# yilundu/cross_attention_renderer

Hardware: AMD Instinct MI355X
Metric: rendered_rays_per_sec (higher is better)
Workload: dtype f32 (split-f16 x3 MFMA); 1 GPU; 256x256 query frame, 64 samples/view, 2 context views (config 2), a new query pose every step (cameras on the host), 1 forward call(s) x 1 scene(s) x 65536 rays per rank; builder_kept=False, H=256, samples_per_view=64, parallelism=one GPU

## Files before the change

### cross_attention_renderer_amd/csrc/car_raychain.hip

```cpp
#include "car_common.h"
#include "car_geom.h"

namespace {

typedef float f32x16 __attribute__((ext_vector_type(16)));
typedef _Float16 half8 __attribute__((ext_vector_type(8)));
typedef __fp16 fp16x2 __attribute__((ext_vector_type(2)));
typedef __attribute__((address_space(3))) void lds_void;

constexpr int kTileFloats = 1024;
constexpr int kMaxNT = 9;
constexpr int kBufFloats = kMaxNT * kTileFloats;
constexpr int kMaxChunks = 96;
constexpr int kMaxLayers = 16;

struct Chunk { unsigned off; int nt; };
struct ChainArgs {
    const float* arena;
    const float* bias;
    const float* scale;
    int layer[kMaxLayers];
    Chunk chunk[kMaxChunks];
    int n_chunks;
    const float* x0; int ld0;
    const float* x1; int ld1;
    const float* z1_in;
    float* out0;
    float* out1;
    const CarRay* rays;
    long M;
    int V, R;
    float zscale;
};

constexpr int kRing = 3;
struct Stream {
    const ChainArgs& a;
    float* lds;
    int g;
    __device__ __forceinline__ float* buffer(int gi) const { return lds + (gi % kRing) * kBufFloats; }
    __device__ __forceinline__ void issue(int gi, int tid, int wave) const {
        if (gi >= a.n_chunks) return;
        const Chunk c = a.chunk[gi];
        const float* src = a.arena + c.off;
        float* dst = buffer(gi);
        for (int t = 0; t < c.nt; ++t) {
            const unsigned lds_dst = __builtin_amdgcn_readfirstlane((unsigned)(uintptr_t)(lds_void*)(dst + 4 * (t * 256 + wave * 64)));
            const float* gsrc = src + 4 * (t * 256 + tid);
            unsigned keep;
            asm volatile("s_mov_b32 %0, m0\n\ts_mov_b32 m0, %2\n\ts_nop 0\n\tglobal_load_lds_dwordx4 %1, off\n\ts_mov_b32 m0, %0"
                         : "=&s"(keep) : "v"(gsrc), "s"(lds_dst) : "memory");
        }
    }
    __device__ __forceinline__ void landed(int gi) const {
        const int n = __builtin_amdgcn_readfirstlane(gi + 1 < a.n_chunks ? a.chunk[gi + 1].nt : 0);
        switch (n) {
            case 1: asm volatile("s_waitcnt vmcnt(1)" ::: "memory"); break;
            case 4: asm volatile("s_waitcnt vmcnt(4)" ::: "memory"); break;
            case 9: asm volatile("s_waitcnt vmcnt(9)" ::: "memory"); break;
            default: asm volatile("s_waitcnt vmcnt(0)" ::: "memory"); break;
        }
        __syncthreads();
    }
    __device__ __forceinline__ void sync() const { landed(g + 1); }
};

#include "car_split.h"
template <int NT>
__device__ __forceinline__ void scale(f32x16 (&acc)[NT], float f) {
#pragma unroll
    for (int t = 0; t < NT; ++t) acc[t] *= f;
}

template <int NT>
__device__ __forceinline__ void mma_chunk(f32x16 (&acc)[NT], const float* wl, const float (&x8)[2][8], float p) {
    half8 bhi[2], blo[2];
#pragma unroll
    for (int kg = 0; kg < 2; ++kg) split8(x8[kg], p, bhi[kg], blo[kg]);
    auto read = [&](int i, half8& ah, half8& al) {
        const int t = i >> 1, kg = i & 1;
        ah = __builtin_bit_cast(half8, *reinterpret_cast<const float4*>(wl + t * kTileFloats + ((kg * 2 + 0) * 64) * 4));
        al = __builtin_bit_cast(half8, *reinterpret_cast<const float4*>(wl + t * kTileFloats + ((kg * 2 + 1) * 64) * 4));
    };
    half8 ah[2], al[2];
    read(0, ah[0], al[0]);
#pragma unroll
    for (int i = 0; i < 2 * NT; ++i) {
        const int t = i >> 1, kg = i & 1, cur = i & 1;
        if (i + 1 < 2 * NT) read(i + 1, ah[cur ^ 1], al[cur ^ 1]);
        __builtin_amdgcn_sched_barrier(0);
        acc[t] = __builtin_amdgcn_mfma_f32_32x32x16_f16(ah[cur], bhi[kg], acc[t], 0, 0, 0);
        acc[t] = __builtin_amdgcn_mfma_f32_32x32x16_f16(ah[cur], blo[kg], acc[t], 0, 0, 0);
        acc[t] = __builtin_amdgcn_mfma_f32_32x32x16_f16(al[cur], bhi[kg], acc[t], 0, 0, 0);
        __builtin_amdgcn_sched_barrier(0);
    }
}

template <int NT>
__device__ __forceinline__ void layer_global(f32x16 (&acc)[NT], const float* xrow, int K, int chunks, float dW, Stream& st, int tid, int lane,
                                             int wave) {
    const int h = lane >> 5;
    auto load = [&](int c, float (&x8)[2][8]) {
#pragma unroll
        for (int kg = 0; kg < 2; ++kg) {
            const int k0 = 32 * c + 16 * kg + 8 * h;
#pragma unroll
            for (int q = 0; q < 2; ++q) {
                const int kq = k0 + 4 * q;
                const float4 v = *reinterpret_cast<const float4*>(xrow + (kq + 4 <= K ? kq : 0));
                const float e[4] = {v.x, v.y, v.z, v.w};
#pragma unroll
                for (int i = 0; i < 4; ++i) x8[kg][4 * q + i] = kq + 4 <= K ? e[i] : (kq + i < K ? xrow[kq + i] : 0.0f);
            }
        }
    };
    float m = 0.0f;
    for (int c = 0; c < chunks; ++c) {
        float x8[2][8];
        load(c, x8);
#pragma unroll
        for (int kg = 0; kg < 2; ++kg)
#pragma unroll
            for (int e = 0; e < 8; ++e) m = fmaxf(m, fabsf(x8[kg][e]));
    }
    m = fmaxf(m, __shfl_xor(m, 32, 64));
    float p, pinv;
    pow2_scale(fmaxf(m, 1e-30f), p, pinv);
    scale<NT>(acc, p / dW);
    float cur[2][8], nxt[2][8];
    load(0, cur);
    for (int c = 0; c < chunks; ++c) {
        st.issue(st.g + 2, tid, wave);
        if (c + 1 < chunks) load(c + 1, nxt);
        mma_chunk<NT>(acc, st.buffer(st.g) + 4 * lane, cur, p);
#pragma unroll
        for (int kg = 0; kg < 2; ++kg)
#pragma unroll
            for (int e = 0; e < 8; ++e) cur[kg][e] = nxt[kg][e];
        st.sync();
        ++st.g;
    }
    scale<NT>(acc, dW * pinv);
}
template <int NSRC, int NT, bool RELU>
__device__ __forceinline__ void layer_chained(f32x16 (&acc)[NT], const f32x16 (&src)[NSRC], float dW, Stream& st, int tid, int lane, int wave) {
    float m = 0.0f;
#pragma unroll
    for (int T = 0; T < NSRC; ++T)
#pragma unroll
        for (int r = 0; r < 16; ++r) m = fmaxf(m, RELU ? src[T][r] : fabsf(src[T][r]));
    m = fmaxf(m, __shfl_xor(m, 32, 64));
    float p, pinv;
    pow2_scale(fmaxf(m, 1e-30f), p, pinv);
    scale<NT>(acc, p / dW);
#pragma unroll
    for (int T = 0; T < NSRC; ++T) {
        st.issue(st.g + 2, tid, wave);
        float x8[2][8];
#pragma unroll
        for (int kg = 0; kg < 2; ++kg)
#pragma unroll
            for (int e = 0; e < 8; ++e) x8[kg][e] = RELU ? fmaxf(src[T][8 * kg + e], 0.0f) : src[T][8 * kg + e];
        mma_chunk<NT>(acc, st.buffer(st.g) + 4 * lane, x8, p);
        st.sync();
        ++st.g;
    }
    scale<NT>(acc, dW * pinv);
}
template <int NT>
__device__ __forceinline__ void add_bias(f32x16 (&acc)[NT], const float* b, int h) {
#pragma unroll
    for (int t = 0; t < NT; ++t)
#pragma unroll
        for (int r = 0; r < 16; ++r) acc[t][r] += b[32 * t + (r & 3) + 8 * (r >> 2) + 4 * h];
}
template <int NT>
__device__ __forceinline__ void zero(f32x16 (&acc)[NT]) {
#pragma unroll
    for (int t = 0; t < NT; ++t)
#pragma unroll
        for (int r = 0; r < 16; ++r) acc[t][r] = 0.0f;
}
template <int NT>
__device__ __forceinline__ void store_rows(const f32x16 (&acc)[NT], float* row, int N, int h) {
#pragma unroll
    for (int t = 0; t < NT; ++t)
#pragma unroll
        for (int g = 0; g < 4; ++g) {
            const int n0 = 32 * t + 8 * g + 4 * h;
            if (n0 + 4 <= N) *reinterpret_cast<float4*>(row + n0) = make_float4(acc[t][4 * g], acc[t][4 * g + 1], acc[t][4 * g + 2], acc[t][4 * g + 3]);
        }
}

__global__ void __launch_bounds__(256, 1) ray_mid_kernel(const ChainArgs a) {
    extern __shared__ __attribute__((aligned(16))) float lds[];
    const int tid = threadIdx.x, lane = tid & 63, wave = tid >> 6, s = lane & 31, h = lane >> 5;
    const long row = (long)blockIdx.x * 128 + wave * 32 + s;
    const long lrow = row < a.M ? row : a.M - 1;
    auto dW = [&](int i) { return a.scale[kMaxLayers + a.layer[i]]; };
    Stream st{a, lds, 0};
    st.issue(0, tid, wave);
    st.issue(1, tid, wave);
    st.landed(0);
    f32x16 z1[9];
    zero<9>(z1);
    add_bias<9>(z1, a.bias, h);
    layer_global<9>(z1, a.x0 + lrow * a.ld0, 576, 18, dW(0), st, tid, lane, wave);
    if (row < a.M) store_rows<9>(z1, a.out0 + row * 288, 288, h);
    f32x16 hb[4];
    zero<4>(hb);
    add_bias<4>(hb, a.bias + 288, h);
    layer_chained<9, 4, false>(hb, z1, dW(1), st, tid, lane, wave);
    f32x16 uh[4];
    zero<4>(uh);
    layer_chained<4, 4, false>(uh, hb, dW(2), st, tid, lane, wave);
    if (row < a.M) store_rows<4>(uh, a.out1 + row * 128, 128, h);
}

__global__ void __launch_bounds__(256, 1) ray_tail_kernel(const ChainArgs a) {
    extern __shared__ __attribute__((aligned(16))) float lds[];
    const int tid = threadIdx.x, lane = tid & 63, wave = tid >> 6, s = lane & 31, h = lane >> 5;
    const long row = (long)blockIdx.x * 128 + wave * 32 + s;
    const long lrow = row < a.M ? row : a.M - 1;
    auto dW = [&](int i) { return a.scale[kMaxLayers + a.layer[i]]; };
    Stream st{a, lds, 0};
    st.issue(0, tid, wave);
    st.issue(1, tid, wave);
    st.landed(0);
    f32x16 z[9];
#pragma unroll
    for (int t = 0; t < 9; ++t)
#pragma unroll
        for (int g = 0; g < 4; ++g) {
            const float4 v = *reinterpret_cast<const float4*>(a.z1_in + lrow * 288 + 32 * t + 8 * g + 4 * h);
            z[t][4 * g] = a.zscale * v.x; z[t][4 * g + 1] = a.zscale * v.y; z[t][4 * g + 2] = a.zscale * v.z; z[t][4 * g + 3] = a.zscale * v.w;
        }
    add_bias<9>(z, a.bias, h);
    layer_global<9>(z, a.x0 + lrow * a.ld0, 576, 18, dW(0), st, tid, lane, wave);
    const float* bias = a.bias + 288;
    f32x16 x[4], net[4];
    zero<4>(x);
    add_bias<4>(x, bias, h);
    layer_global<4>(x, a.x1 + lrow * a.ld1, 18, 1, dW(1), st, tid, lane, wave);
#pragma unroll
    for (int i = 0; i < 3; ++i) {
        add_bias<4>(x, bias + (3 * i + 1) * 128, h);
        layer_chained<9, 4, false>(x, z, dW(2 + 3 * i), st, tid, lane, wave);
        zero<4>(net);
        add_bias<4>(net, bias + (3 * i + 2) * 128, h);
        layer_chained<4, 4, true>(net, x, dW(3 + 3 * i), st, tid, lane, wave);
        add_bias<4>(x, bias + (3 * i + 3) * 128, h);
        layer_chained<4, 4, true>(x, net, dW(4 + 3 * i), st, tid, lane, wave);
    }
    f32x16 o[1];
    zero<1>(o);
    add_bias<1>(o, bias + 10 * 128, h);
    layer_chained<4, 1, true>(o, x, dW(11), st, tid, lane, wave);
    if (row < a.M && h == 0) {
        const long sc = row / a.R, r = row % a.R;
        float ov = 0.0f;
        for (int v = 0; v < a.V; ++v) ov = fmaxf(ov, a.rays[(sc * a.V + v) * a.R + r].overlaps);
        const float valid = ov > 0.0f ? 1.0f : 0.0f;
        for (int k = 0; k < 3; ++k) a.out0[3 * row + k] = o[0][k] * valid + (1.0f - valid);
        a.out1[row] = valid;
    }
}

__global__ void chain_scale_kernel(const float* __restrict__ W, int ldw, const float* __restrict__ W2, int K, int N, float* __restrict__ scale, int slot) {
    __shared__ float red[16];
    float m = 0.0f;
    for (long idx = threadIdx.x; idx < (long)N * K; idx += blockDim.x) {
        const long at = (idx / K) * ldw + idx % K;
        m = fmaxf(m, fabsf(W[at] + (W2 ? W2[at] : 0.0f)));
    }
    for (int o = 32; o > 0; o >>= 1) m = fmaxf(m, __shfl_xor(m, o, 64));
    if ((threadIdx.x & 63) == 0) red[threadIdx.x >> 6] = m;
    __syncthreads();
    if (threadIdx.x == 0) {
        for (int w = 1; w < (int)(blockDim.x / 64); ++w) m = fmaxf(m, red[w]);
        float p, inv;
        pow2_scale(fmaxf(m, 1e-30f), p, inv);
        scale[slot] = p;
        scale[kMaxLayers + slot] = inv;
    }
}
__global__ void pack_chain_kernel(const float* __restrict__ W, int ldw, const float* __restrict__ W2, int K, int N, int tiles, int chained,
                                  long total, const float* __restrict__ scale, int slot, _Float16* __restrict__ packed) {
    const float p = scale[slot];
    for (long idx = (long)blockIdx.x * blockDim.x + threadIdx.x; idx < total; idx += (long)gridDim.x * blockDim.x) {
        const int e = (int)(idx & 7), lane = (int)((idx >> 3) & 63), hl = (int)((idx >> 9) & 1), kg = (int)((idx >> 10) & 1);
        const long ct = idx >> 11;
        const int tile = (int)(ct % tiles), chunk = (int)(ct / tiles);
        const int n = 32 * tile + (lane & 31);
        const int k = chained ? 32 * chunk + (e & 3) + 8 * (2 * kg + (e >> 2)) + 4 * (lane >> 5) : 32 * chunk + 16 * kg + 8 * (lane >> 5) + e;
        float v = 0.0f;
        if (n < N && k < K) v = (W[(long)n * ldw + k] + (W2 ? W2[(long)n * ldw + k] : 0.0f)) * p;
        const _Float16 hi = (_Float16)v;
        packed[idx] = hl == 0 ? hi : (_Float16)(v - (float)hi);
    }
}

}

extern "C" size_t car_chain_packed_floats(int K, int N) { return (size_t)((K + 31) / 32) * ((N + 31) / 32) * kTileFloats; }
extern "C" int car_chain_pack(const float* W, int ldw, const float* W2, int K, int N, int chained, float* packed, float* scale, int slot,
                              void* stream) {
    CAR_REQUIRE(W && packed && scale && K > 0 && N > 0 && ldw >= K && slot >= 0 && slot < kMaxLayers, "car_chain_pack: bad arguments");
    const int tiles = (N + 31) / 32;
    const long total = (long)car_chain_packed_floats(K, N) * 2;
    (void)hipGetLastError();
    hipLaunchKernelGGL(chain_scale_kernel, dim3(1), dim3(1024), 0, (hipStream_t)stream, W, ldw, W2, K, N, scale, slot);
    hipLaunchKernelGGL(pack_chain_kernel, dim3(256), dim3(256), 0, (hipStream_t)stream, W, ldw, W2, K, N, tiles, chained, total, scale, slot,
                       reinterpret_cast<_Float16*>(packed));
    CAR_CHECK_LAUNCH("car_chain_pack");
    return CAR_OK;
}

namespace {
int launch_chain(bool tail, const float* arena, const unsigned* offs, const int* nts, int n_chunks, const float* bias, const float* scale,
                 const int* layers, int n_layers, const float* x0, int ld0, const float* x1, int ld1, const float* z1_in, float* out0, float* out1,
                 const float* rays, long M, int V, int R, float zscale, void* stream) {
    CAR_REQUIRE(n_chunks > 0 && n_chunks <= kMaxChunks && n_layers == (tail ? 12 : 3), "car_ray_chain: %d weight chunks, %d layers", n_chunks, n_layers);
    ChainArgs a;
    a.arena = arena; a.bias = bias; a.scale = scale; a.n_chunks = n_chunks;
    for (int i = 0; i < kMaxLayers; ++i) a.layer[i] = i < n_layers ? layers[i] : 0;
    for (int i = 0; i < n_layers; ++i) CAR_REQUIRE(layers[i] >= 0 && layers[i] < kMaxLayers, "car_ray_chain: bad scale slot");
    for (int i = 0; i < n_chunks; ++i) { a.chunk[i].off = offs[i]; a.chunk[i].nt = nts[i]; }
    a.x0 = x0; a.ld0 = ld0; a.x1 = x1; a.ld1 = ld1; a.z1_in = z1_in; a.out0 = out0; a.out1 = out1; a.rays = (const CarRay*)rays;
    a.M = M; a.V = V; a.R = R; a.zscale = zscale;
    const size_t lds_bytes = (size_t)kRing * kBufFloats * sizeof(float);
    auto kern = tail ? ray_tail_kernel : ray_mid_kernel;
    hipError_t e = hipFuncSetAttribute((const void*)kern, hipFuncAttributeMaxDynamicSharedMemorySize, (int)lds_bytes);
    if (e != hipSuccess) { car_set_error("car_ray_chain: cannot reserve LDS: %s", hipGetErrorString(e)); return CAR_E_LAUNCH; }
    (void)hipGetLastError();
    hipLaunchKernelGGL(kern, dim3(car_div_up(M, 128)), dim3(256), lds_bytes, (hipStream_t)stream, a);
    CAR_CHECK_LAUNCH("car_ray_chain");
    return CAR_OK;
}
}

extern "C" int car_ray_mid(const float* arena, const unsigned* offs, const int* nts, int n_chunks, const float* bias, const float* scale,
                           const int* layers, int n_layers, const float* ebar, int ld_ebar, float* z1, float* uh, long M, void* stream) {
    CAR_REQUIRE(arena && offs && nts && bias && scale && layers && ebar && z1 && uh && M > 0 && ld_ebar >= 576 && ld_ebar % 4 == 0,
                "car_ray_mid: bad arguments");
    return launch_chain(false, arena, offs, nts, n_chunks, bias, scale, layers, n_layers, ebar, ld_ebar, nullptr, 0, nullptr, z1, uh, nullptr, M, 0, 1,
                        0.0f, stream);
}
extern "C" int car_ray_tail(const float* arena, const unsigned* offs, const int* nts, int n_chunks, const float* bias, const float* scale,
                            const int* layers, int n_layers, const float* ebar, int ld_ebar, const float* phi_x, int ld_phi, const float* z1,
                            const float* rays, int b, int V, int R, float* rgb, float* valid, void* stream) {
    CAR_REQUIRE(arena && offs && nts && bias && scale && layers && ebar && phi_x && z1 && rays && rgb && valid, "car_ray_tail: null pointer");
    CAR_REQUIRE(b > 0 && V > 0 && R > 0 && ld_ebar >= 576 && ld_ebar % 4 == 0 && ld_phi >= 20 && ld_phi % 4 == 0, "car_ray_tail: bad sizes");
    return launch_chain(true, arena, offs, nts, n_chunks, bias, scale, layers, n_layers, ebar, ld_ebar, phi_x, ld_phi, z1, rgb, valid, rays, (long)b * R, V,
                        R, (float)V, stream);
}
```

### cross_attention_renderer_amd/csrc/car_render.hip

```cpp
#include "car_common.h"
#include "car_geom.h"
#include <math.h>
#include <string.h>
#include <vector>

namespace {

#include "car_fused_layout.h"

constexpr int kPhiIn = 18, kPhiLd = 20, kBlocks = 3;

inline size_t up64(size_t x) { return (x + 63) & ~(size_t)63; }

struct Plan {
    size_t steps, blob, fbias, wpt, r2qw, r2qb, proj[CAR_MAX_LEVELS], proj16[CAR_MAX_LEVELS], latent_value, lin_in, enc_c, qreh_c, lz_c[kBlocks], fc0_c[kBlocks],
        fc1_c[kBlocks], lout_c, chain_scale, mid_bias, tail_bias, total;
};
inline bool level_on_f16_pipe(int c) { return c % 4 == 0 && c >= 32; }
Plan plan_layout(const car_dims& d) {
    Plan p;
    size_t o = 0;
    auto take = [&](size_t n) { const size_t at = o; o += up64(n); return at; };
    p.steps = take((size_t)d.P);
    p.blob = take(car_fused_blob_floats());
    p.fbias = take(car_fused_bias_floats());
    p.wpt = take((size_t)kC * 4);
    p.r2qw = take(car_round2q_packed_floats());
    p.r2qb = take(car_round2q_bias_floats());
    for (int l = 0; l < CAR_MAX_LEVELS; ++l) p.proj[l] = l < d.n_levels ? take(car_linear_packed_floats(d.level_c[l], kC)) : 0;
    for (int l = 0; l < CAR_MAX_LEVELS; ++l) p.proj16[l] = (l < d.n_levels && level_on_f16_pipe(d.level_c[l])) ? take(car_linear_x3_packed_floats(d.level_c[l], kC)) : 0;
    p.latent_value = take(car_chain_packed_floats(kC, kE));
    p.lin_in = take(car_chain_packed_floats(kPhiIn, kD));
    p.enc_c = take(car_chain_packed_floats(kE, kD));
    p.qreh_c = take(car_chain_packed_floats(kD, kD));
    for (int i = 0; i < kBlocks; ++i) {
        p.lz_c[i] = take(car_chain_packed_floats(kE, kD));
        p.fc0_c[i] = take(car_chain_packed_floats(kD, kD));
        p.fc1_c[i] = take(car_chain_packed_floats(kD, kD));
    }
    p.lout_c = take(car_chain_packed_floats(kD, 3));
    p.chain_scale = take(32);
    p.mid_bias = take(kE + kD);
    p.tail_bias = take(kE + kD + 3 * kBlocks * kD + 32);
    p.total = o;
    return p;
}

int check_dims(const car_dims* d, const char* who) {
    CAR_REQUIRE(d, "%s: null dims", who);
    CAR_REQUIRE(d->b > 0 && d->R > 0 && d->P > 1 && d->H > 1 && d->W > 1, "%s: bad sizes", who);
    CAR_REQUIRE(d->V == 2 && d->n_levels == 3, "%s: the one-call forward covers n_view = 2 and three pyramid levels (got %d, %d); "
                "other configurations run through the stage entries", who, d->V, d->n_levels);
    int csum = 0;
    for (int l = 0; l < d->n_levels; ++l) {
        CAR_REQUIRE(d->level_h[l] > 0 && d->level_w[l] > 0 && d->level_c[l] > 0, "%s: bad level %d", who, l);
        csum += d->level_c[l];
    }
    CAR_REQUIRE(csum == kC, "%s: the levels' channels must add up to %d (got %d)", who, kC, csum);
    CAR_REQUIRE(2 * d->P <= 128 * 3, "%s: too many samples per ray", who);
    CAR_REQUIRE(car_lattice_of(*d).ok, "%s: every pyramid level must be an integer factor coarser than the widest one, the same factor in both "
                "directions (the fused kernel gathers them from their common lattice); other pyramids run through the stage entries", who);
    return CAR_OK;
}

struct Span { size_t off, cnt; };
struct Work {
    Span rays, phi_x, e, g, logit, logit2, pt, pixel_val, coords, at_wt, at_wt2, amax, depth, ebar, z1, uh, valid, part;
    size_t total;
};
const struct { const char* name; Span Work::*buf; } kFindable[] = {
    {"rays", &Work::rays}, {"e", &Work::e}, {"g", &Work::g}, {"logit", &Work::logit}, {"logit2", &Work::logit2}, {"pt", &Work::pt},
    {"at_wt2", &Work::at_wt2}, {"ebar", &Work::ebar}, {"z1", &Work::z1}, {"uh", &Work::uh}, {"part", &Work::part}};
inline size_t step_groups(const car_dims& d) { const int ts = car_fused_tile_steps(); return (size_t)((d.P + ts - 1) / ts); }
Work work_layout(const car_dims& d) {
    Work w;
    size_t o = 0;
    auto take = [&](size_t n) { const Span s{o, n}; o += up64(n); return s; };
    const size_t n = (size_t)d.b * d.V, S = n * d.R * d.P, BR = (size_t)d.b * d.R;
    w.rays = take(n * d.R * CAR_RAY_FLOATS);
    w.phi_x = take(BR * kPhiLd);
    w.e = take(S * kC);
    w.g = take(S * CAR_G_DIM);
    w.logit = take(S);
    w.logit2 = take(S);
    w.pt = take(S * 3);
    w.pixel_val = take(S * 2);
    w.coords = take(n * d.R * 9);
    w.at_wt = take(S);
    w.at_wt2 = take(S);
    w.amax = take(n * d.R);
    w.depth = take(BR);
    w.ebar = take(BR * kC);
    w.z1 = take(BR * kE);
    w.uh = take(BR * kD);
    w.valid = take(BR);
    w.part = take(n * d.R * step_groups(d) * kC);
    w.total = o;
    return w;
}

struct StageRec { const char* name; hipEvent_t start, stop; };
struct Profile {
    bool on = false;
    std::vector<StageRec> recs;
    std::vector<hipEvent_t> pool;
    hipEvent_t event() {
        if (!pool.empty()) { hipEvent_t e = pool.back(); pool.pop_back(); return e; }
        hipEvent_t e = nullptr;
        if (hipEventCreate(&e) != hipSuccess) e = nullptr;
        return e;
    }
    void clear() {
        for (StageRec& r : recs) { pool.push_back(r.start); pool.push_back(r.stop); }
        recs.clear();
    }
};
thread_local Profile g_prof;
struct Stage {
    hipStream_t st;
    bool live;
    Stage(const char* name, hipStream_t s) : st(s), live(g_prof.on) {
        if (!live) return;
        StageRec r{name, g_prof.event(), g_prof.event()};
        if (!r.start || !r.stop) { live = false; return; }
        (void)hipEventRecord(r.start, st);
        g_prof.recs.push_back(r);
    }
    ~Stage() { if (live) (void)hipEventRecord(g_prof.recs.back().stop, st); }
};

}

extern "C" void car_profile_enable(int on) { g_prof.clear(); g_prof.on = on != 0; }
extern "C" void car_profile_reset(void) { g_prof.clear(); }
extern "C" int car_profile_count(void) { return (int)g_prof.recs.size(); }
extern "C" int car_profile_read(int i, const char** name, float* ms) {
    CAR_REQUIRE(i >= 0 && i < (int)g_prof.recs.size() && name && ms, "car_profile_read: no stage %d", i);
    const StageRec& r = g_prof.recs[i];
    if (hipEventSynchronize(r.stop) != hipSuccess || hipEventElapsedTime(ms, r.start, r.stop) != hipSuccess) {
        car_set_error("car_profile_read: %s", hipGetErrorString(hipGetLastError()));
        return CAR_E_LAUNCH;
    }
    *name = r.name;
    return CAR_OK;
}

extern "C" void car_linspace(float a, float b, int n, float* out) {
    if (n == 1) { out[0] = a; return; }
    const float step = (b - a) / (float)(n - 1);
    const int half = n / 2;
    for (int i = 0; i < n; ++i) out[i] = i < half ? a + step * (float)i : b - step * (float)(n - 1 - i);
}

extern "C" size_t car_plan_bytes(const car_dims* dims) {
    if (check_dims(dims, "car_plan_bytes") != CAR_OK) return 0;
    return plan_layout(*dims).total * sizeof(float);
}
extern "C" size_t car_workspace_bytes(const car_dims* dims) {
    if (check_dims(dims, "car_workspace_bytes") != CAR_OK) return 0;
    return work_layout(*dims).total * sizeof(float);
}

namespace {
size_t lattice_floats(const car_dims& d) { const car_lattice L = car_lattice_of(d); return (size_t)d.b * d.V * 2 * L.h * L.w * kC; }
size_t level_floats(const car_dims& d, int l) { return (size_t)d.b * d.V * d.level_h[l] * d.level_w[l] * kC; }
size_t level_offset(const car_dims& d, int level) {
    size_t n = up64(lattice_floats(d)) + 64;
    for (int l = 0; l < level && l < d.n_levels; ++l) n += up64(level_floats(d, l));
    return n;
}
}
extern "C" size_t car_gmeta_offset(const car_dims* dims) {
    if (check_dims(dims, "car_gmeta_offset") != CAR_OK) return 0;
    return up64(lattice_floats(*dims));
}
extern "C" size_t car_gmaps_floats(const car_dims* dims) {
    if (check_dims(dims, "car_gmaps_floats") != CAR_OK) return 0;
    return level_offset(*dims, CAR_MAX_LEVELS + 1);
}
extern "C" int car_lattice_shape(const car_dims* dims, int* lat_h, int* lat_w, int* lat_pad) {
    CAR_TRY(check_dims(dims, "car_lattice_shape"));
    CAR_REQUIRE(lat_h && lat_w && lat_pad, "car_lattice_shape: null pointer");
    const car_lattice L = car_lattice_of(*dims);
    *lat_h = L.h; *lat_w = L.w; *lat_pad = L.pad;
    return CAR_OK;
}
extern "C" int car_workspace_find(const car_dims* dims, const char* name, size_t* offset_floats, size_t* n_floats) {
    CAR_TRY(check_dims(dims, "car_workspace_find"));
    CAR_REQUIRE(name && offset_floats && n_floats, "car_workspace_find: null pointer");
    const Work w = work_layout(*dims);
    for (const auto& t : kFindable)
        if (strcmp(t.name, name) == 0) { *offset_floats = (w.*t.buf).off; *n_floats = (w.*t.buf).cnt; return CAR_OK; }
    car_set_error("car_workspace_find: unknown tensor '%s'", name);
    return CAR_E_ARG;
}

extern "C" int car_plan_build(const car_dims* dims, const car_weights* w, void* plan, void* stream) {
    CAR_TRY(check_dims(dims, "car_plan_build"));
    CAR_REQUIRE(w && plan, "car_plan_build: null pointer");
    const float* const* all = reinterpret_cast<const float* const*>(w);
    for (size_t k = 0; k < sizeof(car_weights) / sizeof(const float*); ++k)
        CAR_REQUIRE(all[k], "car_plan_build: weight pointer %zu of car_weights is null", k);
    CAR_REQUIRE(car_fused_blob_floats() == (size_t)kBlobTiles * kTile && car_fused_bias_floats() == (size_t)(kBiasFloats + kBiasScratch),
                "car_plan_build: the fused kernel was built with another weight layout");
    const Plan p = plan_layout(*dims);
    float* base = static_cast<float*>(plan);
    hipStream_t st = (hipStream_t)stream;
    {
        float steps[1024];
        CAR_REQUIRE(dims->P <= 1024, "car_plan_build: P too large");
        car_linspace(0.0f, 1.0f, dims->P, steps);
        if (hipMemcpyAsync(base + p.steps, steps, sizeof(float) * dims->P, hipMemcpyHostToDevice, st) != hipSuccess ||
            hipStreamSynchronize(st) != hipSuccess) {
            car_set_error("car_plan_build: upload failed: %s", hipGetErrorString(hipGetLastError()));
            return CAR_E_LAUNCH;
        }
    }
    CAR_TRY(car_fused_pack(w, base + p.blob, base + p.fbias, base + p.wpt, stream));
    CAR_TRY(car_round2q_pack(w->query_repeat_embed_w, w->query_repeat_embed_b, w->query_repeat_embed_2_w, w->query_repeat_embed_2_b,
                             w->query_embed_w, w->query_embed_b, w->query_embed_2_w, w->query_embed_2_b, base + p.r2qw, base + p.r2qb, stream));
    int coff = 0;
    for (int l = 0; l < dims->n_levels; ++l) {
        CAR_TRY(car_linear_pack(w->query_encode_latent_w + coff, kC + 3, nullptr, dims->level_c[l], kC, base + p.proj[l], stream));
        if (level_on_f16_pipe(dims->level_c[l]))
            CAR_TRY(car_linear_x3_pack(w->query_encode_latent_w + coff, kC + 3, dims->level_c[l], kC, base + p.proj16[l], stream));
        coff += dims->level_c[l];
    }
    float* cs = base + p.chain_scale;
    CAR_TRY(car_chain_pack(w->latent_value_w, kC, nullptr, kC, kE, 0, base + p.latent_value, cs, 0, stream));
    CAR_TRY(car_chain_pack(w->encode_latent_w, kE, nullptr, kE, kD, 1, base + p.enc_c, cs, 1, stream));
    CAR_TRY(car_chain_pack(w->query_repeat_embed_w, kD + 16, nullptr, kD, kD, 1, base + p.qreh_c, cs, 2, stream));
    CAR_TRY(car_chain_pack(w->phi_lin_in_w, kPhiIn, nullptr, kPhiIn, kD, 0, base + p.lin_in, cs, 3, stream));
    for (int i = 0; i < kBlocks; ++i) {
        CAR_TRY(car_chain_pack(w->phi_lin_z_w[i], 2 * kE, w->phi_lin_z_w[i] + kE, kE, kD, 1, base + p.lz_c[i], cs, 4 + 3 * i, stream));
        CAR_TRY(car_chain_pack(w->phi_fc_0_w[i], kD, nullptr, kD, kD, 1, base + p.fc0_c[i], cs, 5 + 3 * i, stream));
        CAR_TRY(car_chain_pack(w->phi_fc_1_w[i], kD, nullptr, kD, kD, 1, base + p.fc1_c[i], cs, 6 + 3 * i, stream));
    }
    CAR_TRY(car_chain_pack(w->phi_lin_out_w, kD, nullptr, kD, 3, 1, base + p.lout_c, cs, 13, stream));
    const int tail_floats = kE + kD + 3 * kBlocks * kD + 32;
    if (hipMemsetAsync(base + p.tail_bias, 0, sizeof(float) * tail_floats, st) != hipSuccess) { car_set_error("car_plan_build: memset failed"); return CAR_E_LAUNCH; }
    auto d2d = [&](float* dst, const float* src, int n) { return hipMemcpyAsync(dst, src, sizeof(float) * n, hipMemcpyDeviceToDevice, st) == hipSuccess; };
    bool ok = d2d(base + p.mid_bias, w->latent_value_b, kE) && d2d(base + p.mid_bias + kE, w->encode_latent_b, kD);
    float* tb = base + p.tail_bias;
    ok = ok && d2d(tb, w->latent_value_b, kE) && d2d(tb + kE, w->phi_lin_in_b, kD);
    tb += kE + kD;
    for (int i = 0; i < kBlocks; ++i)
        ok = ok && d2d(tb + (3 * i + 0) * kD, w->phi_lin_z_b[i], kD) && d2d(tb + (3 * i + 1) * kD, w->phi_fc_0_b[i], kD) &&
             d2d(tb + (3 * i + 2) * kD, w->phi_fc_1_b[i], kD);
    ok = ok && d2d(tb + 3 * kBlocks * kD, w->phi_lin_out_b, 3);
    if (!ok) { car_set_error("car_plan_build: bias copy failed"); return CAR_E_LAUNCH; }
    return CAR_OK;
}

struct Plan16 { size_t blob, fbias, wpt, total; };
Plan16 plan16_layout() {
    Plan16 p;
    size_t o = 0;
    auto take = [&](size_t n) { const size_t at = o; o += up64(n); return at; };
    p.blob = take(car_fused_blob16_floats());
    p.fbias = take(car_fused_bias_floats());
    p.wpt = take((size_t)kC * 4);
    p.total = o;
    return p;
}
extern "C" size_t car_plan_f16_bytes(const car_dims* dims) {
    if (check_dims(dims, "car_plan_f16_bytes") != CAR_OK) return 0;
    return plan16_layout().total * sizeof(float);
}
extern "C" int car_plan_f16_build(const car_dims* dims, const car_weights* w, void* plan16, void* stream) {
    CAR_TRY(check_dims(dims, "car_plan_f16_build"));
    CAR_REQUIRE(w && plan16, "car_plan_f16_build: null pointer");
    CAR_REQUIRE(car_fused_blob16_floats() == (size_t)kBlobTiles * kTileHi && car_fused_bias_floats() == (size_t)(kBiasFloats + kBiasScratch),
                "car_plan_f16_build: the fused kernel was built with another weight layout");
    const Plan16 p = plan16_layout();
    float* base = static_cast<float*>(plan16);
    return car_fused_pack_hi(w, base + p.blob, base + p.fbias, base + p.wpt, stream);
}

extern "C" int car_project_maps(const car_dims* dims, const void* plan, const float* const* maps, float* gmaps, void* stream) {
    CAR_TRY(check_dims(dims, "car_project_maps"));
    CAR_REQUIRE(plan && maps && gmaps, "car_project_maps: null pointer");
    const Plan p = plan_layout(*dims);
    const float* base = static_cast<const float*>(plan);
    hipStream_t st = (hipStream_t)stream;
    float* gmeta = gmaps + car_gmeta_offset(dims);
    if (hipMemsetAsync(gmeta, 0, sizeof(float) * CAR_MAX_LEVELS, st) != hipSuccess) { car_set_error("car_project_maps: memset failed"); return CAR_E_LAUNCH; }
    const car_lattice L = car_lattice_of(*dims);
    const float* lv[CAR_MAX_LEVELS];
    for (int l = 0; l < dims->n_levels; ++l) {
        CAR_REQUIRE(maps[l], "car_project_maps: level %d is null", l);
        const long M = (long)dims->b * dims->V * dims->level_h[l] * dims->level_w[l];
        float* gl = gmaps + level_offset(*dims, l);
        if (level_on_f16_pipe(dims->level_c[l]) && ((uintptr_t)maps[l] & 15) == 0)
            CAR_TRY(car_linear_x3(maps[l], dims->level_c[l], base + p.proj16[l], nullptr, dims->level_c[l], kC, gl, kC, M, 0, stream));
        else
            CAR_TRY(car_linear(maps[l], dims->level_c[l], base + p.proj[l], dims->level_c[l], kC, gl, kC, M, 0, stream));
        lv[l] = gl;
    }
    return car_launch_merge(lv, dims->level_h, dims->level_w, L.r, dims->n_levels, L.h, L.w, L.pad, dims->b * dims->V, gmaps,
                            reinterpret_cast<unsigned*>(gmeta), st, "car_project_maps (merge)");
}

static int render_phases(const char* entry, const car_dims* dims, const void* plan, const car_inputs* in, const car_outputs* out,
                         void* workspace, size_t workspace_bytes, int phases, void* stream, const void* plan16 = nullptr) {
    const int which = phases & ~CAR_PHASE_ROWS_FIRST_ROUND;
    CAR_REQUIRE(which == CAR_PHASE_SAMPLES || which == CAR_PHASE_RAYS || which == (CAR_PHASE_SAMPLES | CAR_PHASE_RAYS),
                "%s: phases = %d (CAR_PHASE_SAMPLES, CAR_PHASE_RAYS or both, optionally | CAR_PHASE_ROWS_FIRST_ROUND)", entry, phases);
    CAR_TRY(check_dims(dims, "car_render_forward"));
    CAR_REQUIRE(plan && in && out && workspace, "car_render_forward: null pointer");
    CAR_REQUIRE(in->poses && in->uv && in->lattice && in->gmeta && out->rgb, "car_render_forward: poses, uv, lattice, gmeta and rgb are required");
    const car_dims& d = *dims;
    const Plan p = plan_layout(d);
    const Work w = work_layout(d);
    CAR_REQUIRE(workspace_bytes >= w.total * sizeof(float), "car_render_forward: workspace of %zu bytes, %zu needed", workspace_bytes,
                w.total * sizeof(float));
    const float* pl = static_cast<const float*>(plan);
    float* ws = static_cast<float*>(workspace);
    hipStream_t st = (hipStream_t)stream;
    const int b = d.b, V = d.V, R = d.R, P = d.P;
    const bool rows_first = (phases & CAR_PHASE_ROWS_FIRST_ROUND) != 0;
    CAR_REQUIRE(!d.no_sample || in->steps, "car_render_forward: no_sample needs `steps` (the P depths along the query ray, models.py:221-222)");
    const float* steps = in->steps ? in->steps : pl + p.steps;
    const long BR = (long)b * R;
    float* coords = out->coords ? out->coords : ws + w.coords.off;
    float* pixel_val = out->pixel_val ? out->pixel_val : ws + w.pixel_val.off;
    float* at_wt = out->at_wt ? out->at_wt : ws + w.at_wt.off;
    float* depth = out->depth_ray ? out->depth_ray : ws + w.depth.off;
    float* valid = out->valid_mask ? out->valid_mask : ws + w.valid.off;
    int32_t* amax = out->at_wt_max ? out->at_wt_max : reinterpret_cast<int32_t*>(ws + w.amax.off);

    if (phases & CAR_PHASE_SAMPLES) {
    {
        Stage stage("ray_setup", st);
        if (hipMemsetAsync(ws + w.phi_x.off, 0, sizeof(float) * BR * kPhiLd, st) != hipSuccess) { car_set_error("car_render_forward: memset failed"); return CAR_E_LAUNCH; }
        CAR_TRY(car_ray_setup(in->poses, in->uv, b, V, R, d.H, d.W, P, d.no_sample != 0, steps, ws + w.rays.off, coords, ws + w.phi_x.off, kPhiLd, stream));
    }
    {
        Stage stage("fused_samples", st);
        const car_lattice L = car_lattice_of(d);
        if (plan16) {
            const Plan16 q = plan16_layout();
            const float* p16 = static_cast<const float*>(plan16);
            CAR_TRY(car_fused_samples_f16(in->poses, ws + w.rays.off, steps, in->lattice, L.h, L.w, L.pad, in->gmeta, p16 + q.wpt, p16 + q.blob,
                                          p16 + q.fbias, b, V, R, P, d.H, d.W, d.no_sample != 0, ws + w.e.off, ws + w.g.off, ws + w.logit.off, ws + w.pt.off, pixel_val,
                                          rows_first ? nullptr : ws + w.part.off, stream));
        } else if (rows_first)
            CAR_TRY(car_fused_samples(in->poses, ws + w.rays.off, steps, in->lattice, L.h, L.w, L.pad, in->gmeta, pl + p.wpt, pl + p.blob,
                                      pl + p.fbias, b, V, R, P, d.H, d.W, d.no_sample != 0, ws + w.e.off, ws + w.g.off, ws + w.logit.off, ws + w.pt.off, pixel_val, stream));
        else
            CAR_TRY(car_fused_samples_parts(in->poses, ws + w.rays.off, steps, in->lattice, L.h, L.w, L.pad, in->gmeta, pl + p.wpt, pl + p.blob,
                                            pl + p.fbias, b, V, R, P, d.H, d.W, d.no_sample != 0, ws + w.e.off, ws + w.g.off, ws + w.logit.off, ws + w.pt.off, pixel_val,
                                            ws + w.part.off, stream));
    }
    }
    if (!(phases & CAR_PHASE_RAYS)) return CAR_OK;
    {
        Stage stage("attend_1", st);
        if (rows_first)
            CAR_TRY(car_attend(ws + w.logit.off, nullptr, kD, ws + w.e.off, kC, b, V, R, P, nullptr, 0.0f, at_wt, ws + w.ebar.off, kC, 1, ws + w.pt.off, in->poses,
                               depth, amax, stream));
        else
            CAR_TRY(car_attend_parts(ws + w.logit.off, ws + w.part.off, car_fused_tile_steps(), kC, b, V, R, P, at_wt, ws + w.ebar.off, kC, 1, ws + w.pt.off, in->poses,
                                     depth, amax, stream));
    }
    unsigned offs[96];
    int nts[96];
    int nch = 0;
    auto chunks = [&](size_t at, int n, int nt) { for (int c = 0; c < n; ++c) { offs[nch] = (unsigned)(at + (size_t)c * nt * 1024); nts[nch++] = nt; } };
    CAR_REQUIRE(p.total < (1ull << 32), "car_render_forward: plan too large");
    if (d.repeat_attention) {
        {
            Stage stage("ray_layers_1", st);
            nch = 0;
            chunks(p.latent_value, 18, 9); chunks(p.enc_c, 9, 4); chunks(p.qreh_c, 4, 4);
            const int layers[3] = {0, 1, 2};
            CAR_TRY(car_ray_mid(pl, offs, nts, nch, pl + p.mid_bias, pl + p.chain_scale, layers, 3, ws + w.ebar.off, kC, ws + w.z1.off, ws + w.uh.off, BR, stream));
        }
        {
            Stage stage("round2_logits", st);
            CAR_TRY(car_round2_logits_from_g(ws + w.g.off, ws + w.uh.off, pl + p.r2qw, pl + p.r2qb, b, V, R, P, ws + w.logit2.off, stream));
        }
        {
            Stage stage("attend_2", st);
            CAR_TRY(car_attend(ws + w.logit2.off, nullptr, kD, ws + w.e.off, kC, b, V, R, P, nullptr, 0.0f, ws + w.at_wt2.off, ws + w.ebar.off, kC, 1, nullptr,
                               nullptr, nullptr, nullptr, stream));
        }
    } else if (hipMemsetAsync(ws + w.z1.off, 0, sizeof(float) * BR * kE, st) != hipSuccess) {
        car_set_error("car_render_forward: memset failed");
        return CAR_E_LAUNCH;
    }
    {
        Stage stage("ray_layers_2", st);
        nch = 0;
        chunks(p.latent_value, 18, 9); chunks(p.lin_in, 1, 4);
        for (int i = 0; i < kBlocks; ++i) { chunks(p.lz_c[i], 9, 4); chunks(p.fc0_c[i], 4, 4); chunks(p.fc1_c[i], 4, 4); }
        chunks(p.lout_c, 4, 1);
        const int layers[12] = {0, 3, 4, 5, 6, 7, 8, 9, 10, 11, 12, 13};
        CAR_TRY(car_ray_tail(pl, offs, nts, nch, pl + p.tail_bias, pl + p.chain_scale, layers, 12, ws + w.ebar.off, kC, ws + w.phi_x.off, kPhiLd, ws + w.z1.off,
                             ws + w.rays.off, b, V, R, out->rgb, valid, stream));
    }
    return CAR_OK;
}

extern "C" int car_render_forward(const car_dims* dims, const void* plan, const car_inputs* in, const car_outputs* out,
                                  void* workspace, size_t workspace_bytes, void* stream) {
    return render_phases("car_render_forward", dims, plan, in, out, workspace, workspace_bytes, CAR_PHASE_SAMPLES | CAR_PHASE_RAYS, stream);
}

extern "C" int car_render_forward_phase(const car_dims* dims, const void* plan, const car_inputs* in, const car_outputs* out,
                                        void* workspace, size_t workspace_bytes, int phases, void* stream) {
    return render_phases("car_render_forward_phase", dims, plan, in, out, workspace, workspace_bytes, phases, stream);
}

extern "C" int car_render_forward_f16(const car_dims* dims, const void* plan, const void* plan16, const car_inputs* in, const car_outputs* out,
                                      void* workspace, size_t workspace_bytes, int phases, void* stream) {
    CAR_REQUIRE(plan16, "car_render_forward_f16: null plan16");
    return render_phases("car_render_forward_f16", dims, plan, in, out, workspace, workspace_bytes, phases, stream, plan16);
}
```

### cross_attention_renderer_amd/csrc/car_round2.hip

```cpp
#include "car_common.h"

namespace {

typedef float f32x16 __attribute__((ext_vector_type(16)));
typedef float f32x4 __attribute__((ext_vector_type(4)));
typedef _Float16 half8 __attribute__((ext_vector_type(8)));
typedef __fp16 fp16x2 __attribute__((ext_vector_type(2)));
constexpr int kD = 128, kNT = 4, kTile = 1024, kChunks = 4;
constexpr int kWaves = 8, kStageLd = 36;
constexpr int kLdsW1 = kChunks * kNT * kTile;
constexpr int kLdsBias = kLdsW1 + kNT * 512;
constexpr int kLdsStage = kLdsBias + 2 * kD + 4;
constexpr size_t kLdsBytes = (size_t)(kLdsStage + kWaves * 32 * kStageLd) * sizeof(float);
constexpr int kLdsWq1 = kLdsBias;
constexpr int kLdsBiasG = kLdsWq1 + kNT * 512;
constexpr int kBiasFloatsG = 4 * kD + 8;
constexpr int kScratchG = kD * kD;
constexpr size_t kLdsBytesG = (size_t)(kLdsBiasG + kBiasFloatsG) * sizeof(float);

#include "car_split.h"

template <bool ZERO = false>
__device__ __forceinline__ void first_layer(const half8& ghi, const half8& glo, const float* lw1, const float* lb1, float up, int lane, int h,
                                            f32x16 (&ug)[kNT]) {
#pragma unroll
    for (int t = 0; t < kNT; ++t) {
#pragma unroll
        for (int r = 0; r < 16; ++r) ug[t][r] = ZERO ? 0.0f : lb1[32 * t + (r & 3) + 8 * (r >> 2) + 4 * h] * up;
        const float* w1 = lw1 + t * 512 + 4 * lane;
        const half8 ah = __builtin_bit_cast(half8, *reinterpret_cast<const float4*>(w1));
        const half8 al = __builtin_bit_cast(half8, *reinterpret_cast<const float4*>(w1 + 256));
        ug[t] = __builtin_amdgcn_mfma_f32_32x32x16_f16(ah, ghi, ug[t], 0, 0, 0);
        ug[t] = __builtin_amdgcn_mfma_f32_32x32x16_f16(ah, glo, ug[t], 0, 0, 0);
        ug[t] = __builtin_amdgcn_mfma_f32_32x32x16_f16(al, ghi, ug[t], 0, 0, 0);
    }
}
template <bool ZERO = false>
__device__ __forceinline__ void second_layer(const f32x16 (&x)[kNT], float xp, const float* lw2, const float* lb2, float up2, int lane, int h,
                                             f32x16 (&acc)[kNT]) {
#pragma unroll
    for (int t = 0; t < kNT; ++t)
#pragma unroll
        for (int r = 0; r < 16; ++r) acc[t][r] = ZERO ? 0.0f : lb2[32 * t + (r & 3) + 8 * (r >> 2) + 4 * h] * up2;
#pragma unroll
    for (int c = 0; c < kChunks; ++c) {
        half8 bhi[2], blo[2];
#pragma unroll
        for (int kg = 0; kg < 2; ++kg) {
            float x8[8];
#pragma unroll
            for (int e = 0; e < 8; ++e) x8[e] = x[c][8 * kg + e];
            split8(x8, xp, bhi[kg], blo[kg]);
        }
        const float* wl = lw2 + c * kNT * kTile + 4 * lane;
        auto read = [&](int i, half8& ah, half8& al) {
            const int t = i >> 1, kg = i & 1;
            ah = __builtin_bit_cast(half8, *reinterpret_cast<const float4*>(wl + t * kTile + ((kg * 2 + 0) * 64) * 4));
            al = __builtin_bit_cast(half8, *reinterpret_cast<const float4*>(wl + t * kTile + ((kg * 2 + 1) * 64) * 4));
        };
        half8 ah[2], al[2];
        read(0, ah[0], al[0]);
#pragma unroll
        for (int i = 0; i < 2 * kNT; ++i) {
            const int t = i >> 1, kg = i & 1, cur = i & 1;
            if (i + 1 < 2 * kNT) read(i + 1, ah[cur ^ 1], al[cur ^ 1]);
            __builtin_amdgcn_sched_barrier(0);
            acc[t] = __builtin_amdgcn_mfma_f32_32x32x16_f16(ah[cur], bhi[kg], acc[t], 0, 0, 0);
            acc[t] = __builtin_amdgcn_mfma_f32_32x32x16_f16(ah[cur], blo[kg], acc[t], 0, 0, 0);
            acc[t] = __builtin_amdgcn_mfma_f32_32x32x16_f16(al[cur], bhi[kg], acc[t], 0, 0, 0);
            __builtin_amdgcn_sched_barrier(0);
        }
    }
}

template <bool G>
__global__ void __launch_bounds__(512) round2_kernel(const float* __restrict__ g, const float* __restrict__ uh,
                                                     const float* __restrict__ qry, const float* __restrict__ wpacked,
                                                     const float* __restrict__ bias, int V, int R, int P, long S,
                                                     float* __restrict__ logit) {
    extern __shared__ __attribute__((aligned(16))) float lds[];
    const int tid = threadIdx.x, lane = tid & 63, wave = tid >> 6;
    const int s = lane & 31, h = lane >> 5;
    const int qd = lane & 7, r8 = lane >> 3;
    constexpr int kW = G ? kLdsBiasG : kLdsBias, kB = G ? kBiasFloatsG : 2 * kD + 4;
    for (int k = tid; k < kW / 4; k += 512)
        *reinterpret_cast<float4*>(lds + 4 * k) = *reinterpret_cast<const float4*>(wpacked + 4 * k);
    for (int k = tid; k < kB; k += 512) lds[kW + k] = bias[k];
    __syncthreads();
    const float* lb = lds + kW;
    const float down1 = lb[(G ? 4 : 2) * kD], down2 = lb[(G ? 4 : 2) * kD + 1];
    float* stage = lds + kLdsStage + wave * 32 * kStageLd;

    for (long row0 = ((long)blockIdx.x * kWaves + wave) * 32; row0 < S; row0 += (long)gridDim.x * kWaves * 32) {
        float4 qs[G ? 1 : kChunks][G ? 1 : 4];
        if constexpr (!G) {
#pragma unroll
            for (int it = 0; it < 4; ++it) {
                const long row = row0 + r8 + 8 * it < S ? row0 + r8 + 8 * it : S - 1;
#pragma unroll
                for (int c = 0; c < kChunks; ++c) {
                    const f32x4 v = __builtin_nontemporal_load(reinterpret_cast<const f32x4*>(qry + row * kD + 32 * c + 4 * qd));
                    qs[c][it] = make_float4(v[0], v[1], v[2], v[3]);
                }
            }
        }
        const long srow = row0 + s < S ? row0 + s : S - 1;
        const long nr = srow / P;
        const float* uhrow = uh + (((nr / R) / V) * R + nr % R) * kD;
        half8 ghi, glo;
        float gp, ginv;
        {
            const float4 g0 = *reinterpret_cast<const float4*>(g + srow * 16 + 8 * h);
            const float4 g1 = *reinterpret_cast<const float4*>(g + srow * 16 + 8 * h + 4);
            const float gx[8] = {g0.x, g0.y, g0.z, g0.w, g1.x, g1.y, g1.z, g1.w};
            float m = 0.0f;
#pragma unroll
            for (int k = 0; k < 8; ++k) m = fmaxf(m, fabsf(gx[k]));
            m = fmaxf(m, __shfl_xor(m, 32, 64));
            pow2_scale(fmaxf(m, 1e-30f), gp, ginv);
            split8(gx, gp, ghi, glo);
        }
        f32x16 ug[kNT];
        first_layer<G>(ghi, glo, lds + kLdsW1, lb, gp / down1, lane, h, ug);
        const float undo1 = down1 * ginv;
        float xm = 0.0f;
#pragma unroll
        for (int t = 0; t < kNT; ++t)
#pragma unroll
            for (int gq = 0; gq < 4; ++gq) {
                const float4 u = *reinterpret_cast<const float4*>(uhrow + 32 * t + 8 * gq + 4 * h);
                float uu[4] = {u.x, u.y, u.z, u.w};
                if constexpr (G) {
                    const float4 b = *reinterpret_cast<const float4*>(lb + 32 * t + 8 * gq + 4 * h);
                    uu[0] += b.x; uu[1] += b.y; uu[2] += b.z; uu[3] += b.w;
                }
#pragma unroll
                for (int r = 0; r < 4; ++r) {
                    const float x = fmaxf(fmaf(ug[t][4 * gq + r], undo1, uu[r]), 0.0f);
                    ug[t][4 * gq + r] = x;
                    xm = fmaxf(xm, x);
                }
            }
        float dot = 0.0f;
        if constexpr (G) {
            const float downq = lb[4 * kD + 2];
            f32x16 xq[kNT];
            first_layer<true>(ghi, glo, lds + kLdsWq1, lb + 2 * kD, gp / downq, lane, h, xq);
            const float undoq = downq * ginv;
            const float* lu = lb + 3 * kD;
            const float* lq = lb + 2 * kD;
            float xqm = 0.0f, dot_u = 0.0f;
#pragma unroll
            for (int t = 0; t < kNT; ++t)
#pragma unroll
                for (int gq = 0; gq < 4; ++gq) {
                    const float4 u = *reinterpret_cast<const float4*>(lu + 32 * t + 8 * gq + 4 * h);
                    const float4 b = *reinterpret_cast<const float4*>(lq + 32 * t + 8 * gq + 4 * h);
                    const float uu[4] = {u.x, u.y, u.z, u.w}, bb[4] = {b.x, b.y, b.z, b.w};
#pragma unroll
                    for (int r = 0; r < 4; ++r) {
                        const float x = fmaxf(fmaf(xq[t][4 * gq + r], undoq, bb[r]), 0.0f);
                        xq[t][4 * gq + r] = x;
                        xqm = fmaxf(xqm, x);
                        dot_u = fmaf(uu[r], x, dot_u);
                    }
                }
            xqm = fmaxf(xqm, __shfl_xor(xqm, 32, 64));
            float xp, xinv;
            pow2_scale(fmaxf(xqm, 1e-30f), xp, xinv);
            f32x16 acc[kNT];
            second_layer<true>(xq, xp, lds, lb + kD, xp / down2, lane, h, acc);
            const float* lv = lb + kD;
            float dot_v = 0.0f;
#pragma unroll
            for (int t = 0; t < kNT; ++t)
#pragma unroll
                for (int gq = 0; gq < 4; ++gq) {
                    const float4 v4 = *reinterpret_cast<const float4*>(lv + 32 * t + 8 * gq + 4 * h);
                    const float vv[4] = {v4.x, v4.y, v4.z, v4.w};
#pragma unroll
                    for (int r = 0; r < 4; ++r) {
                        dot = fmaf(ug[t][4 * gq + r], acc[t][4 * gq + r], dot);
                        dot_v = fmaf(ug[t][4 * gq + r], vv[r], dot_v);
                    }
                }
            dot = fmaf(dot, down2 * xinv, dot_u + dot_v);
            dot += __shfl_xor(dot, 32, 64);
            dot += lb[4 * kD + 3];
        } else {
            xm = fmaxf(xm, __shfl_xor(xm, 32, 64));
            float xp, xinv;
            pow2_scale(fmaxf(xm, 1e-30f), xp, xinv);
            f32x16 acc[kNT];
            second_layer(ug, xp, lds, lb + kD, xp / down2, lane, h, acc);
#pragma unroll
            for (int t = 0; t < kNT; ++t) {
#pragma unroll
                for (int it = 0; it < 4; ++it) *reinterpret_cast<float4*>(stage + (r8 + 8 * it) * kStageLd + 4 * qd) = qs[t][it];
#pragma unroll
                for (int gq = 0; gq < 4; ++gq) {
                    const float4 qv = *reinterpret_cast<const float4*>(stage + s * kStageLd + 8 * gq + 4 * h);
                    dot = fmaf(acc[t][4 * gq + 0], qv.x, dot); dot = fmaf(acc[t][4 * gq + 1], qv.y, dot);
                    dot = fmaf(acc[t][4 * gq + 2], qv.z, dot); dot = fmaf(acc[t][4 * gq + 3], qv.w, dot);
                }
            }
            dot += __shfl_xor(dot, 32, 64);
            dot *= down2 * xinv;
        }
        if (h == 0 && row0 + s < S) logit[row0 + s] = dot / 16.0f;
    }
}

}

extern "C" size_t car_round2_packed_floats(void) { return (size_t)kLdsBias; }
extern "C" size_t car_round2_bias_floats(void) { return (size_t)(2 * kD + 4); }

extern "C" size_t car_round2q_packed_floats(void) { return (size_t)kLdsBiasG; }
extern "C" size_t car_round2q_bias_floats(void) { return (size_t)(kBiasFloatsG + kScratchG); }

static int launch_round2(bool qg, const float* g, const float* uh, const float* qry, const float* wpacked, const float* bias,
                         int b, int V, int R, int P, float* logit, void* stream, const char* who) {
    CAR_REQUIRE(g && uh && (qg || qry) && wpacked && bias && logit, "%s: null pointer", who);
    CAR_REQUIRE(b > 0 && V > 0 && R > 0 && P > 0, "%s: bad sizes", who);
    const long S = (long)b * V * R * P;
    void (*kern)(const float*, const float*, const float*, const float*, const float*, int, int, int, long, float*) =
        qg ? round2_kernel<true> : round2_kernel<false>;
    const size_t lds_bytes = qg ? kLdsBytesG : kLdsBytes;
    hipError_t e = hipFuncSetAttribute((const void*)kern, hipFuncAttributeMaxDynamicSharedMemorySize, (int)lds_bytes);
    if (e != hipSuccess) { car_set_error("%s: cannot reserve LDS: %s", who, hipGetErrorString(e)); return CAR_E_LAUNCH; }
    const long groups = (S + 255) / 256;
    const unsigned blocks = (unsigned)(groups < 1024 ? groups : 1024);
    (void)hipGetLastError();
    hipLaunchKernelGGL(kern, dim3(blocks), dim3(512), lds_bytes, (hipStream_t)stream, g, uh, qry, wpacked, bias, V, R, P, S, logit);
    hipError_t e_ = hipGetLastError();
    if (e_ != hipSuccess) { car_set_error("%s: launch failed: %s", who, hipGetErrorString(e_)); return CAR_E_LAUNCH; }
    return CAR_OK;
}

extern "C" int car_round2_logits(const float* g, const float* uh, const float* qry, const float* wpacked, const float* bias,
                                 int b, int V, int R, int P, float* logit, void* stream) {
    return launch_round2(false, g, uh, qry, wpacked, bias, b, V, R, P, logit, stream, "car_round2_logits");
}

extern "C" int car_round2_logits_from_g(const float* g, const float* uh, const float* wpacked, const float* bias, int b, int V, int R, int P,
                                        float* logit, void* stream) {
    return launch_round2(true, g, uh, nullptr, wpacked, bias, b, V, R, P, logit, stream, "car_round2_logits_from_g");
}
```

Before: 2.154 million rays/s.

## Switch ray chain to 16x16 MFMA tiles with 8 waves and restructure round2 query path

Result: no change. 2.161 million rays/s (median of 4 runs) (+0.3%).

```diff
diff --git a/cross_attention_renderer_amd/csrc/car_raychain.hip b/cross_attention_renderer_amd/csrc/car_raychain.hip
--- a/cross_attention_renderer_amd/csrc/car_raychain.hip
+++ b/cross_attention_renderer_amd/csrc/car_raychain.hip
@@ -3,13 +3,14 @@
 
 namespace {
 
-typedef float f32x16 __attribute__((ext_vector_type(16)));
+typedef float f32x4 __attribute__((ext_vector_type(4)));
 typedef _Float16 half8 __attribute__((ext_vector_type(8)));
 typedef __fp16 fp16x2 __attribute__((ext_vector_type(2)));
 typedef __attribute__((address_space(3))) void lds_void;
 
-constexpr int kTileFloats = 1024;
-constexpr int kMaxNT = 9;
+constexpr int kTileFloats = 512;
+constexpr int kMaxNT = 18;
+constexpr int kWaves = 8, kWaveRays = 16, kGroupRays = kWaves * kWaveRays;
 constexpr int kBufFloats = kMaxNT * kTileFloats;
 constexpr int kMaxChunks = 96;
 constexpr int kMaxLayers = 16;
@@ -38,26 +39,30 @@
     const ChainArgs& a;
     float* lds;
     int g;
+    int wave;
     __device__ __forceinline__ float* buffer(int gi) const { return lds + (gi % kRing) * kBufFloats; }
-    __device__ __forceinline__ void issue(int gi, int tid, int wave) const {
+    __device__ __forceinline__ int wave_loads(int gi, int wave) const { return gi < a.n_chunks ? (2 * a.chunk[gi].nt - wave + kWaves - 1) / kWaves : 0; }
+    __device__ __forceinline__ void issue(int gi, int lane, int wave) const {
         if (gi >= a.n_chunks) return;
         const Chunk c = a.chunk[gi];
         const float* src = a.arena + c.off;
         float* dst = buffer(gi);
-        for (int t = 0; t < c.nt; ++t) {
-            const unsigned lds_dst = __builtin_amdgcn_readfirstlane((unsigned)(uintptr_t)(lds_void*)(dst + 4 * (t * 256 + wave * 64)));
-            const float* gsrc = src + 4 * (t * 256 + tid);
+        for (int j = wave; j < 2 * c.nt; j += kWaves) {
+            const unsigned lds_dst = __builtin_amdgcn_readfirstlane((unsigned)(uintptr_t)(lds_void*)(dst + 4 * (j * 64)));
+            const float* gsrc = src + 4 * (j * 64 + lane);
             unsigned keep;
             asm volatile("s_mov_b32 %0, m0\n\ts_mov_b32 m0, %2\n\ts_nop 0\n\tglobal_load_lds_dwordx4 %1, off\n\ts_mov_b32 m0, %0"
                          : "=&s"(keep) : "v"(gsrc), "s"(lds_dst) : "memory");
         }
     }
     __device__ __forceinline__ void landed(int gi) const {
-        const int n = __builtin_amdgcn_readfirstlane(gi + 1 < a.n_chunks ? a.chunk[gi + 1].nt : 0);
+        const int n = __builtin_amdgcn_readfirstlane(wave_loads(gi + 1, wave));
         switch (n) {
             case 1: asm volatile("s_waitcnt vmcnt(1)" ::: "memory"); break;
+            case 2: asm volatile("s_waitcnt vmcnt(2)" ::: "memory"); break;
+            case 3: asm volatile("s_waitcnt vmcnt(3)" ::: "memory"); break;
             case 4: asm volatile("s_waitcnt vmcnt(4)" ::: "memory"); break;
-            case 9: asm volatile("s_waitcnt vmcnt(9)" ::: "memory"); break;
+            case 5: asm volatile("s_waitcnt vmcnt(5)" ::: "memory"); break;
             default: asm volatile("s_waitcnt vmcnt(0)" ::: "memory"); break;
         }
         __syncthreads();
@@ -67,100 +72,97 @@
 
 #include "car_split.h"
 template <int NT>
-__device__ __forceinline__ void scale(f32x16 (&acc)[NT], float f) {
+__device__ __forceinline__ void scale(f32x4 (&acc)[NT], float f) {
 #pragma unroll
     for (int t = 0; t < NT; ++t) acc[t] *= f;
 }
 
 template <int NT>
-__device__ __forceinline__ void mma_chunk(f32x16 (&acc)[NT], const float* wl, const float (&x8)[2][8], float p) {
-    half8 bhi[2], blo[2];
-#pragma unroll
-    for (int kg = 0; kg < 2; ++kg) split8(x8[kg], p, bhi[kg], blo[kg]);
-    auto read = [&](int i, half8& ah, half8& al) {
-        const int t = i >> 1, kg = i & 1;
-        ah = __builtin_bit_cast(half8, *reinterpret_cast<const float4*>(wl + t * kTileFloats + ((kg * 2 + 0) * 64) * 4));
-        al = __builtin_bit_cast(half8, *reinterpret_cast<const float4*>(wl + t * kTileFloats + ((kg * 2 + 1) * 64) * 4));
+__device__ __forceinline__ void mma_chunk(f32x4 (&acc)[NT], const float* wl, const float (&x8)[8], float p) {
+    half8 bhi, blo;
+    split8(x8, p, bhi, blo);
+    auto read = [&](int t, half8& ah, half8& al) {
+        ah = __builtin_bit_cast(half8, *reinterpret_cast<const float4*>(wl + t * kTileFloats));
+        al = __builtin_bit_cast(half8, *reinterpret_cast<const float4*>(wl + t * kTileFloats + 256));
     };
-    half8 ah[2], al[2];
+    half8 ah[3], al[3];
     read(0, ah[0], al[0]);
-#pragma unroll
-    for (int i = 0; i < 2 * NT; ++i) {
-        const int t = i >> 1, kg = i & 1, cur = i & 1;
-        if (i + 1 < 2 * NT) read(i + 1, ah[cur ^ 1], al[cur ^ 1]);
+    if (NT > 1) read(1, ah[1], al[1]);
+#pragma unroll
+    for (int t = 0; t < NT; ++t) {
+        const int cur = t % 3;
+        if (t + 2 < NT) read(t + 2, ah[(t + 2) % 3], al[(t + 2) % 3]);
         __builtin_amdgcn_sched_barrier(0);
-        acc[t] = __builtin_amdgcn_mfma_f32_32x32x16_f16(ah[cur], bhi[kg], acc[t], 0, 0, 0);
-        acc[t] = __builtin_amdgcn_mfma_f32_32x32x16_f16(ah[cur], blo[kg], acc[t], 0, 0, 0);
-        acc[t] = __builtin_amdgcn_mfma_f32_32x32x16_f16(al[cur], bhi[kg], acc[t], 0, 0, 0);
+        acc[t] = __builtin_amdgcn_mfma_f32_16x16x32_f16(ah[cur], bhi, acc[t], 0, 0, 0);
+        acc[t] = __builtin_amdgcn_mfma_f32_16x16x32_f16(ah[cur], blo, acc[t], 0, 0, 0);
+        acc[t] = __builtin_amdgcn_mfma_f32_16x16x32_f16(al[cur], bhi, acc[t], 0, 0, 0);
         __builtin_amdgcn_sched_barrier(0);
     }
 }
-
-template <int NT>
-__device__ __forceinline__ void layer_global(f32x16 (&acc)[NT], const float* xrow, int K, int chunks, float dW, Stream& st, int tid, int lane,
-                                             int wave) {
-    const int h = lane >> 5;
-    auto load = [&](int c, float (&x8)[2][8]) {
-#pragma unroll
-        for (int kg = 0; kg < 2; ++kg) {
-            const int k0 = 32 * c + 16 * kg + 8 * h;
-#pragma unroll
-            for (int q = 0; q < 2; ++q) {
-                const int kq = k0 + 4 * q;
-                const float4 v = *reinterpret_cast<const float4*>(xrow + (kq + 4 <= K ? kq : 0));
-                const float e[4] = {v.x, v.y, v.z, v.w};
-#pragma unroll
-                for (int i = 0; i < 4; ++i) x8[kg][4 * q + i] = kq + 4 <= K ? e[i] : (kq + i < K ? xrow[kq + i] : 0.0f);
-            }
+__device__ __forceinline__ float ray_max(float m) {
+    m = fmaxf(m, __shfl_xor(m, 16, 64));
+    return fmaxf(m, __shfl_xor(m, 32, 64));
+}
+
+template <int NT>
+__device__ __forceinline__ void layer_global(f32x4 (&acc)[NT], const float* xrow, int K, int chunks, float dW, Stream& st, int lane) {
+    const int q = lane >> 4;
+    auto load = [&](int c, float (&x8)[8]) {
+        const int k0 = 32 * c + 8 * q;
+#pragma unroll
+        for (int j = 0; j < 2; ++j) {
+            const int kq = k0 + 4 * j;
+            const float4 v = *reinterpret_cast<const float4*>(xrow + (kq + 4 <= K ? kq : 0));
+            const float e[4] = {v.x, v.y, v.z, v.w};
+#pragma unroll
+            for (int i = 0; i < 4; ++i) x8[4 * j + i] = kq + 4 <= K ? e[i] : (kq + i < K ? xrow[kq + i] : 0.0f);
         }
     };
     float m = 0.0f;
     for (int c = 0; c < chunks; ++c) {
-        float x8[2][8];
+        float x8[8];
         load(c, x8);
 #pragma unroll
-        for (int kg = 0; kg < 2; ++kg)
-#pragma unroll
-            for (int e = 0; e < 8; ++e) m = fmaxf(m, fabsf(x8[kg][e]));
-    }
-    m = fmaxf(m, __shfl_xor(m, 32, 64));
+        for (int e = 0; e < 8; ++e) m = fmaxf(m, fabsf(x8[e]));
+    }
+    m = ray_max(m);
     float p, pinv;
     pow2_scale(fmaxf(m, 1e-30f), p, pinv);
     scale<NT>(acc, p / dW);
-    float cur[2][8], nxt[2][8];
+    float cur[8], nxt[8];
     load(0, cur);
     for (int c = 0; c < chunks; ++c) {
-        st.issue(st.g + 2, tid, wave);
+        st.issue(st.g + 2, lane, st.wave);
         if (c + 1 < chunks) load(c + 1, nxt);
         mma_chunk<NT>(acc, st.buffer(st.g) + 4 * lane, cur, p);
 #pragma unroll
-        for (int kg = 0; kg < 2; ++kg)
-#pragma unroll
-            for (int e = 0; e < 8; ++e) cur[kg][e] = nxt[kg][e];
+        for (int e = 0; e < 8; ++e) cur[e] = nxt[e];
         st.sync();
         ++st.g;
     }
     scale<NT>(acc, dW * pinv);
 }
 template <int NSRC, int NT, bool RELU>
-__device__ __forceinline__ void layer_chained(f32x16 (&acc)[NT], const f32x16 (&src)[NSRC], float dW, Stream& st, int tid, int lane, int wave) {
+__device__ __forceinline__ void layer_chained(f32x4 (&acc)[NT], const f32x4 (&src)[NSRC], float dW, Stream& st, int lane) {
+    static_assert(NSRC % 2 == 0, "a K step takes two source tiles");
     float m = 0.0f;
 #pragma unroll
     for (int T = 0; T < NSRC; ++T)
 #pragma unroll
-        for (int r = 0; r < 16; ++r) m = fmaxf(m, RELU ? src[T][r] : fabsf(src[T][r]));
-    m = fmaxf(m, __shfl_xor(m, 32, 64));
+        for (int r = 0; r < 4; ++r) m = fmaxf(m, RELU ? src[T][r] : fabsf(src[T][r]));
+    m = ray_max(m);
     float p, pinv;
     pow2_scale(fmaxf(m, 1e-30f), p, pinv);
     scale<NT>(acc, p / dW);
 #pragma unroll
-    for (int T = 0; T < NSRC; ++T) {
-        st.issue(st.g + 2, tid, wave);
-        float x8[2][8];
-#pragma unroll
-        for (int kg = 0; kg < 2; ++kg)
-#pragma unroll
-            for (int e = 0; e < 8; ++e) x8[kg][e] = RELU ? fmaxf(src[T][8 * kg + e], 0.0f) : src[T][8 * kg + e];
+    for (int c = 0; c < NSRC / 2; ++c) {
+        st.issue(st.g + 2, lane, st.wave);
+        float x8[8];
+#pragma unroll
+        for (int e = 0; e < 8; ++e) {
+            const float v = src[2 * c + (e >> 2)][e & 3];
+            x8[e] = RELU ? fmaxf(v, 0.0f) : v;
+        }
         mma_chunk<NT>(acc, st.buffer(st.g) + 4 * lane, x8, p);
         st.sync();
         ++st.g;
@@ -168,95 +170,89 @@
     scale<NT>(acc, dW * pinv);
 }
 template <int NT>
-__device__ __forceinline__ void add_bias(f32x16 (&acc)[NT], const float* b, int h) {
+__device__ __forceinline__ void add_bias(f32x4 (&acc)[NT], const float* b, int q) {
+#pragma unroll
+    for (int t = 0; t < NT; ++t) {
+        const float4 v = *reinterpret_cast<const float4*>(b + 16 * t + 4 * q);
+        acc[t][0] += v.x; acc[t][1] += v.y; acc[t][2] += v.z; acc[t][3] += v.w;
+    }
+}
+template <int NT>
+__device__ __forceinline__ void zero(f32x4 (&acc)[NT]) {
 #pragma unroll
     for (int t = 0; t < NT; ++t)
 #pragma unroll
-        for (int r = 0; r < 16; ++r) acc[t][r] += b[32 * t + (r & 3) + 8 * (r >> 2) + 4 * h];
-}
-template <int NT>
-__device__ __forceinline__ void zero(f32x16 (&acc)[NT]) {
-#pragma unroll
-    for (int t = 0; t < NT; ++t)
-#pragma unroll
-        for (int r = 0; r < 16; ++r) acc[t][r] = 0.0f;
-}
-template <int NT>
-__device__ __forceinline__ void store_rows(const f32x16 (&acc)[NT], float* row, int N, int h) {
-#pragma unroll
-    for (int t = 0; t < NT; ++t)
-#pragma unroll
-        for (int g = 0; g < 4; ++g) {
-            const int n0 = 32 * t + 8 * g + 4 * h;
-            if (n0 + 4 <= N) *reinterpret_cast<float4*>(row + n0) = make_float4(acc[t][4 * g], acc[t][4 * g + 1], acc[t][4 * g + 2], acc[t][4 * g + 3]);
-        }
-}
-
-__global__ void __launch_bounds__(256, 1) ray_mid_kernel(const ChainArgs a) {
+        for (int r = 0; r < 4; ++r) acc[t][r] = 0.0f;
+}
+template <int NT>
+__device__ __forceinline__ void store_rows(const f32x4 (&acc)[NT], float* row, int q) {
+#pragma unroll
+    for (int t = 0; t < NT; ++t) *reinterpret_cast<float4*>(row + 16 * t + 4 * q) = make_float4(acc[t][0], acc[t][1], acc[t][2], acc[t][3]);
+}
+
+__global__ void __launch_bounds__(64 * kWaves) ray_mid_kernel(const ChainArgs a) {
     extern __shared__ __attribute__((aligned(16))) float lds[];
-    const int tid = threadIdx.x, lane = tid & 63, wave = tid >> 6, s = lane & 31, h = lane >> 5;
-    const long row = (long)blockIdx.x * 128 + wave * 32 + s;
+    const int tid = threadIdx.x, lane = tid & 63, wave = __builtin_amdgcn_readfirstlane(tid >> 6), s = lane & 15, q = lane >> 4;
+    const long row = (long)blockIdx.x * kGroupRays + wave * kWaveRays + s;
     const long lrow = row < a.M ? row : a.M - 1;
     auto dW = [&](int i) { return a.scale[kMaxLayers + a.layer[i]]; };
-    Stream st{a, lds, 0};
-    st.issue(0, tid, wave);
-    st.issue(1, tid, wave);
+    Stream st{a, lds, 0, wave};
+    st.issue(0, lane, wave);
+    st.issue(1, lane, wave);
     st.landed(0);
-    f32x16 z1[9];
-    zero<9>(z1);
-    add_bias<9>(z1, a.bias, h);
-    layer_global<9>(z1, a.x0 + lrow * a.ld0, 576, 18, dW(0), st, tid, lane, wave);
-    if (row < a.M) store_rows<9>(z1, a.out0 + row * 288, 288, h);
-    f32x16 hb[4];
-    zero<4>(hb);
-    add_bias<4>(hb, a.bias + 288, h);
-    layer_chained<9, 4, false>(hb, z1, dW(1), st, tid, lane, wave);
-    f32x16 uh[4];
-    zero<4>(uh);
-    layer_chained<4, 4, false>(uh, hb, dW(2), st, tid, lane, wave);
-    if (row < a.M) store_rows<4>(uh, a.out1 + row * 128, 128, h);
-}
-
-__global__ void __launch_bounds__(256, 1) ray_tail_kernel(const ChainArgs a) {
+    f32x4 z1[18];
+    zero<18>(z1);
+    add_bias<18>(z1, a.bias, q);
+    layer_global<18>(z1, a.x0 + lrow * a.ld0, 576, 18, dW(0), st, lane);
+    if (row < a.M) store_rows<18>(z1, a.out0 + row * 288, q);
+    f32x4 hb[8];
+    zero<8>(hb);
+    add_bias<8>(hb, a.bias + 288, q);
+    layer_chained<18, 8, false>(hb, z1, dW(1), st, lane);
+    f32x4 uh[8];
+    zero<8>(uh);
+    layer_chained<8, 8, false>(uh, hb, dW(2), st, lane);
+    if (row < a.M) store_rows<8>(uh, a.out1 + row * 128, q);
+}
+
+__global__ void __launch_bounds__(64 * kWaves) ray_tail_kernel(const ChainArgs a) {
     extern __shared__ __attribute__((aligned(16))) float lds[];
-    const int tid = threadIdx.x, lane = tid & 63, wave = tid >> 6, s = lane & 31, h = lane >> 5;
-    const long row = (long)blockIdx.x * 128 + wave * 32 + s;
+    const int tid = threadIdx.x, lane = tid & 63, wave = __builtin_amdgcn_readfirstlane(tid >> 6), s = lane & 15, q = lane >> 4;
+    const long row = (long)blockIdx.x * kGroupRays + wave * kWaveRays + s;
     const long lrow = row < a.M ? row : a.M - 1;
     auto dW = [&](int i) { return a.scale[kMaxLayers + a.layer[i]]; };
-    Stream st{a, lds, 0};
-    st.issue(0, tid, wave);
-    st.issue(1, tid, wave);
+    Stream st{a, lds, 0, wave};
+    st.issue(0, lane, wave);
+    st.issue(1, lane, wave);
     st.landed(0);
-    f32x16 z[9];
-#pragma unroll
-    for (int t = 0; t < 9; ++t)
-#pragma unroll
-        for (int g = 0; g < 4; ++g) {
-            const float4 v = *reinterpret_cast<const float4*>(a.z1_in + lrow * 288 + 32 * t + 8 * g + 4 * h);
-            z[t][4 * g] = a.zscale * v.x; z[t][4 * g + 1] = a.zscale * v.y; z[t][4 * g + 2] = a.zscale * v.z; z[t][4 * g + 3] = a.zscale * v.w;
-        }
-    add_bias<9>(z, a.bias, h);
-    layer_global<9>(z, a.x0 + lrow * a.ld0, 576, 18, dW(0), st, tid, lane, wave);
+    f32x4 z[18];
+#pragma unroll
+    for (int t = 0; t < 18; ++t) {
+        const float4 v = *reinterpret_cast<const float4*>(a.z1_in + lrow * 288 + 16 * t + 4 * q);
+        z[t][0] = a.zscale * v.x; z[t][1] = a.zscale * v.y; z[t][2] = a.zscale * v.z; z[t][3] = a.zscale * v.w;
+    }
+    add_bias<18>(z, a.bias, q);
+    layer_global<18>(z, a.x0 + lrow * a.ld0, 576, 18, dW(0), st, lane);
     const float* bias = a.bias + 288;
-    f32x16 x[4], net[4];
-    zero<4>(x);
-    add_bias<4>(x, bias, h);
-    layer_global<4>(x, a.x1 + lrow * a.ld1, 18, 1, dW(1), st, tid, lane, wave);
-#pragma unroll
+    f32x4 x[8], net[8];
+    zero<8>(x);
+    add_bias<8>(x, bias, q);
+    layer_global<8>(x, a.x1 + lrow * a.ld1, 18, 1, dW(1), st, lane);
+#pragma unroll 1
     for (int i = 0; i < 3; ++i) {
-        add_bias<4>(x, bias + (3 * i + 1) * 128, h);
-        layer_chained<9, 4, false>(x, z, dW(2 + 3 * i), st, tid, lane, wave);
-        zero<4>(net);
-        add_bias<4>(net, bias + (3 * i + 2) * 128, h);
-        layer_chained<4, 4, true>(net, x, dW(3 + 3 * i), st, tid, lane, wave);
-        add_bias<4>(x, bias + (3 * i + 3) * 128, h);
-        layer_chained<4, 4, true>(x, net, dW(4 + 3 * i), st, tid, lane, wave);
-    }
-    f32x16 o[1];
+        add_bias<8>(x, bias + (3 * i + 1) * 128, q);
+        layer_chained<18, 8, false>(x, z, dW(2 + 3 * i), st, lane);
+        zero<8>(net);
+        add_bias<8>(net, bias + (3 * i + 2) * 128, q);
+        layer_chained<8, 8, true>(net, x, dW(3 + 3 * i), st, lane);
+        add_bias<8>(x, bias + (3 * i + 3) * 128, q);
+        layer_chained<8, 8, true>(x, net, dW(4 + 3 * i), st, lane);
+    }
+    f32x4 o[1];
     zero<1>(o);
-    add_bias<1>(o, bias + 10 * 128, h);
-    layer_chained<4, 1, true>(o, x, dW(11), st, tid, lane, wave);
-    if (row < a.M && h == 0) {
+    add_bias<1>(o, bias + 10 * 128, q);
+    layer_chained<8, 1, true>(o, x, dW(11), st, lane);
+    if (row < a.M && q == 0) {
         const long sc = row / a.R, r = row % a.R;
         float ov = 0.0f;
         for (int v = 0; v < a.V; ++v) ov = fmaxf(ov, a.rays[(sc * a.V + v) * a.R + r].overlaps);
@@ -288,11 +284,11 @@
                                   long total, const float* __restrict__ scale, int slot, _Float16* __restrict__ packed) {
     const float p = scale[slot];
     for (long idx = (long)blockIdx.x * blockDim.x + threadIdx.x; idx < total; idx += (long)gridDim.x * blockDim.x) {
-        const int e = (int)(idx & 7), lane = (int)((idx >> 3) & 63), hl = (int)((idx >> 9) & 1), kg = (int)((idx >> 10) & 1);
-        const long ct = idx >> 11;
+        const int e = (int)(idx & 7), lane = (int)((idx >> 3) & 63), hl = (int)((idx >> 9) & 1);
+        const long ct = idx >> 10;
         const int tile = (int)(ct % tiles), chunk = (int)(ct / tiles);
-        const int n = 32 * tile + (lane & 31);
-        const int k = chained ? 32 * chunk + (e & 3) + 8 * (2 * kg + (e >> 2)) + 4 * (lane >> 5) : 32 * chunk + 16 * kg + 8 * (lane >> 5) + e;
+        const int n = 16 * tile + (lane & 15);
+        const int k = chained ? 32 * chunk + 16 * (e >> 2) + 4 * (lane >> 4) + (e & 3) : 32 * chunk + 8 * (lane >> 4) + e;
         float v = 0.0f;
         if (n < N && k < K) v = (W[(long)n * ldw + k] + (W2 ? W2[(long)n * ldw + k] : 0.0f)) * p;
         const _Float16 hi = (_Float16)v;
@@ -302,11 +298,11 @@
 
 }
 
-extern "C" size_t car_chain_packed_floats(int K, int N) { return (size_t)((K + 31) / 32) * ((N + 31) / 32) * kTileFloats; }
+extern "C" size_t car_chain_packed_floats(int K, int N) { return (size_t)((K + 31) / 32) * ((N + 15) / 16) * kTileFloats; }
 extern "C" int car_chain_pack(const float* W, int ldw, const float* W2, int K, int N, int chained, float* packed, float* scale, int slot,
                               void* stream) {
     CAR_REQUIRE(W && packed && scale && K > 0 && N > 0 && ldw >= K && slot >= 0 && slot < kMaxLayers, "car_chain_pack: bad arguments");
-    const int tiles = (N + 31) / 32;
+    const int tiles = (N + 15) / 16;
     const long total = (long)car_chain_packed_floats(K, N) * 2;
     (void)hipGetLastError();
     hipLaunchKernelGGL(chain_scale_kernel, dim3(1), dim3(1024), 0, (hipStream_t)stream, W, ldw, W2, K, N, scale, slot);
@@ -325,7 +321,10 @@
     a.arena = arena; a.bias = bias; a.scale = scale; a.n_chunks = n_chunks;
     for (int i = 0; i < kMaxLayers; ++i) a.layer[i] = i < n_layers ? layers[i] : 0;
     for (int i = 0; i < n_layers; ++i) CAR_REQUIRE(layers[i] >= 0 && layers[i] < kMaxLayers, "car_ray_chain: bad scale slot");
-    for (int i = 0; i < n_chunks; ++i) { a.chunk[i].off = offs[i]; a.chunk[i].nt = nts[i]; }
+    for (int i = 0; i < n_chunks; ++i) {
+        CAR_REQUIRE(nts[i] > 0 && nts[i] <= kMaxNT, "car_ray_chain: chunk %d has %d tiles", i, nts[i]);
+        a.chunk[i].off = offs[i]; a.chunk[i].nt = nts[i];
+    }
     a.x0 = x0; a.ld0 = ld0; a.x1 = x1; a.ld1 = ld1; a.z1_in = z1_in; a.out0 = out0; a.out1 = out1; a.rays = (const CarRay*)rays;
     a.M = M; a.V = V; a.R = R; a.zscale = zscale;
     const size_t lds_bytes = (size_t)kRing * kBufFloats * sizeof(float);
@@ -333,7 +332,7 @@
     hipError_t e = hipFuncSetAttribute((const void*)kern, hipFuncAttributeMaxDynamicSharedMemorySize, (int)lds_bytes);
     if (e != hipSuccess) { car_set_error("car_ray_chain: cannot reserve LDS: %s", hipGetErrorString(e)); return CAR_E_LAUNCH; }
     (void)hipGetLastError();
-    hipLaunchKernelGGL(kern, dim3(car_div_up(M, 128)), dim3(256), lds_bytes, (hipStream_t)stream, a);
+    hipLaunchKernelGGL(kern, dim3(car_div_up(M, kGroupRays)), dim3(64 * kWaves), lds_bytes, (hipStream_t)stream, a);
     CAR_CHECK_LAUNCH("car_ray_chain");
     return CAR_OK;
 }
diff --git a/cross_attention_renderer_amd/csrc/car_render.hip b/cross_attention_renderer_amd/csrc/car_render.hip
--- a/cross_attention_renderer_amd/csrc/car_render.hip
+++ b/cross_attention_renderer_amd/csrc/car_render.hip
@@ -366,13 +366,13 @@
     unsigned offs[96];
     int nts[96];
     int nch = 0;
-    auto chunks = [&](size_t at, int n, int nt) { for (int c = 0; c < n; ++c) { offs[nch] = (unsigned)(at + (size_t)c * nt * 1024); nts[nch++] = nt; } };
+    auto chunks = [&](size_t at, int n, int nt) { for (int c = 0; c < n; ++c) { offs[nch] = (unsigned)(at + (size_t)c * nt * 512); nts[nch++] = nt; } };
     CAR_REQUIRE(p.total < (1ull << 32), "car_render_forward: plan too large");
     if (d.repeat_attention) {
         {
             Stage stage("ray_layers_1", st);
             nch = 0;
-            chunks(p.latent_value, 18, 9); chunks(p.enc_c, 9, 4); chunks(p.qreh_c, 4, 4);
+            chunks(p.latent_value, 18, 18); chunks(p.enc_c, 9, 8); chunks(p.qreh_c, 4, 8);
             const int layers[3] = {0, 1, 2};
             CAR_TRY(car_ray_mid(pl, offs, nts, nch, pl + p.mid_bias, pl + p.chain_scale, layers, 3, ws + w.ebar.off, kC, ws + w.z1.off, ws + w.uh.off, BR, stream));
         }
@@ -392,8 +392,8 @@
     {
         Stage stage("ray_layers_2", st);
         nch = 0;
-        chunks(p.latent_value, 18, 9); chunks(p.lin_in, 1, 4);
-        for (int i = 0; i < kBlocks; ++i) { chunks(p.lz_c[i], 9, 4); chunks(p.fc0_c[i], 4, 4); chunks(p.fc1_c[i], 4, 4); }
+        chunks(p.latent_value, 18, 18); chunks(p.lin_in, 1, 8);
+        for (int i = 0; i < kBlocks; ++i) { chunks(p.lz_c[i], 9, 8); chunks(p.fc0_c[i], 4, 8); chunks(p.fc1_c[i], 4, 8); }
         chunks(p.lout_c, 4, 1);
         const int layers[12] = {0, 3, 4, 5, 6, 7, 8, 9, 10, 11, 12, 13};
         CAR_TRY(car_ray_tail(pl, offs, nts, nch, pl + p.tail_bias, pl + p.chain_scale, layers, 12, ws + w.ebar.off, kC, ws + w.phi_x.off, kPhiLd, ws + w.z1.off,
diff --git a/cross_attention_renderer_amd/csrc/car_round2.hip b/cross_attention_renderer_amd/csrc/car_round2.hip
--- a/cross_attention_renderer_amd/csrc/car_round2.hip
+++ b/cross_attention_renderer_amd/csrc/car_round2.hip
@@ -70,6 +70,166 @@
             acc[t] = __builtin_amdgcn_mfma_f32_32x32x16_f16(al[cur], bhi[kg], acc[t], 0, 0, 0);
             __builtin_amdgcn_sched_barrier(0);
         }
+    }
+}
+
+template <class Shadow>
+__device__ __forceinline__ void second_layer_tile(const half8 (&bhi)[kChunks][2], const half8 (&blo)[kChunks][2], const float* lw2, int t, int lane, f32x16& acc,
+                                                  Shadow&& shadow) {
+    const float* wl = lw2 + t * kTile + 4 * lane;
+    auto read = [&](int i, half8& ah, half8& al) {
+        const int c = i >> 1, kg = i & 1;
+        ah = __builtin_bit_cast(half8, *reinterpret_cast<const float4*>(wl + c * kNT * kTile + ((kg * 2 + 0) * 64) * 4));
+        al = __builtin_bit_cast(half8, *reinterpret_cast<const float4*>(wl + c * kNT * kTile + ((kg * 2 + 1) * 64) * 4));
+    };
+    half8 ah[2], al[2];
+    read(0, ah[0], al[0]);
+    f32x16 a = {0.0f, 0.0f, 0.0f, 0.0f, 0.0f, 0.0f, 0.0f, 0.0f, 0.0f, 0.0f, 0.0f, 0.0f, 0.0f, 0.0f, 0.0f, 0.0f};
+#pragma unroll
+    for (int i = 0; i < 2 * kChunks; ++i) {
+        const int c = i >> 1, kg = i & 1, cur = i & 1;
+        if (i + 1 < 2 * kChunks) read(i + 1, ah[cur ^ 1], al[cur ^ 1]);
+        __builtin_amdgcn_sched_barrier(0);
+        a = __builtin_amdgcn_mfma_f32_32x32x16_f16(ah[cur], bhi[c][kg], a, 0, 0, 0);
+        __builtin_amdgcn_sched_barrier(0);
+        shadow(3 * i);
+        __builtin_amdgcn_sched_barrier(0);
+        a = __builtin_amdgcn_mfma_f32_32x32x16_f16(ah[cur], blo[c][kg], a, 0, 0, 0);
+        __builtin_amdgcn_sched_barrier(0);
+        shadow(3 * i + 1);
+        __builtin_amdgcn_sched_barrier(0);
+        a = __builtin_amdgcn_mfma_f32_32x32x16_f16(al[cur], bhi[c][kg], a, 0, 0, 0);
+        __builtin_amdgcn_sched_barrier(0);
+        shadow(3 * i + 2);
+        __builtin_amdgcn_sched_barrier(0);
+    }
+    acc = a;
+}
+
+typedef const __attribute__((address_space(3))) float lds_float;
+template <class Ptr>
+__device__ __forceinline__ void load4(Ptr p, float (&v)[4]) {
+    const f32x4 q = *(const f32x4*)p;
+    v[0] = q[0]; v[1] = q[1]; v[2] = q[2]; v[3] = q[3];
+}
+__device__ __forceinline__ void load4(lds_float* p, float (&v)[4]) {
+    const f32x4 q = *(const __attribute__((address_space(3))) f32x4*)p;
+    v[0] = q[0]; v[1] = q[1]; v[2] = q[2]; v[3] = q[3];
+}
+
+__device__ __forceinline__ void round2_g_tiles(const float* __restrict__ g, const float* __restrict__ uh, const float* lds, int V, int R, int P, long S,
+                                               float* __restrict__ logit, int lane, long first, long stride) {
+    const int s = lane & 31, h = lane >> 5;
+    const float* lb = lds + kLdsBiasG;
+    const float down1 = lb[4 * kD], down2 = lb[4 * kD + 1], downq = lb[4 * kD + 2];
+    unsigned lane_tables = (unsigned)(uintptr_t)(lds_float*)(lb + 4 * h);
+    asm volatile("" : "+v"(lane_tables));
+    lds_float* lbh = (lds_float*)(uintptr_t)lane_tables;
+    lds_float* lvh = lbh + kD;
+    lds_float* lqh = lbh + 2 * kD;
+    lds_float* luh = lbh + 3 * kD;
+    const bool narrow = S <= 0x7fffffffL;
+    auto sample = [&](long r0) { return r0 + s < S ? r0 + s : S - 1; };
+    auto uh_row = [&](long srow) {
+        if (narrow) {
+            const unsigned nr = (unsigned)srow / (unsigned)P;
+            return uh + ((size_t)((nr / (unsigned)R) / (unsigned)V) * (unsigned)R + nr % (unsigned)R) * kD;
+        }
+        const long nr = srow / P;
+        return uh + (((nr / R) / V) * R + nr % R) * kD;
+    };
+    if (first >= S) return;
+    long srow = sample(first);
+    float4 g0 = *reinterpret_cast<const float4*>(g + srow * 16 + 8 * h), g1 = *reinterpret_cast<const float4*>(g + srow * 16 + 8 * h + 4);
+    const float* uhrow = uh_row(srow);
+    float un[4][4];
+#pragma unroll
+    for (int gq = 0; gq < 4; ++gq) load4(uhrow + 8 * gq + 4 * h, un[gq]);
+    for (long row0 = first; row0 < S; row0 += stride) {
+        const long nsrow = sample(row0 + stride);
+        const float4 ng0 = *reinterpret_cast<const float4*>(g + nsrow * 16 + 8 * h), ng1 = *reinterpret_cast<const float4*>(g + nsrow * 16 + 8 * h + 4);
+        const float* nuhrow = uh_row(nsrow);
+        half8 ghi, glo;
+        float gp, ginv;
+        {
+            const float gx[8] = {g0.x, g0.y, g0.z, g0.w, g1.x, g1.y, g1.z, g1.w};
+            float m = 0.0f;
+#pragma unroll
+            for (int k = 0; k < 8; ++k) m = fmaxf(m, fabsf(gx[k]));
+            m = fmaxf(m, __shfl_xor(m, 32, 64));
+            pow2_scale(fmaxf(m, 1e-30f), gp, ginv);
+            split8(gx, gp, ghi, glo);
+        }
+        f32x16 xq[kNT];
+        first_layer<true>(ghi, glo, lds + kLdsWq1, lb, gp / downq, lane, h, xq);
+        const float undoq = downq * ginv;
+        float xqm = 0.0f, dot_u = 0.0f;
+#pragma unroll
+        for (int t = 0; t < kNT; ++t)
+#pragma unroll
+            for (int gq = 0; gq < 4; ++gq) {
+                float uu[4], bb[4];
+                load4(luh + 32 * t + 8 * gq, uu);
+                load4(lqh + 32 * t + 8 * gq, bb);
+#pragma unroll
+                for (int r = 0; r < 4; ++r) {
+                    const float x = fmaxf(fmaf(xq[t][4 * gq + r], undoq, bb[r]), 0.0f);
+                    xq[t][4 * gq + r] = x;
+                    xqm = fmaxf(xqm, x);
+                    dot_u = fmaf(uu[r], x, dot_u);
+                }
+            }
+        xqm = fmaxf(xqm, __shfl_xor(xqm, 32, 64));
+        float xp, xinv;
+        pow2_scale(fmaxf(xqm, 1e-30f), xp, xinv);
+        half8 bhi[kChunks][2], blo[kChunks][2];
+#pragma unroll
+        for (int c = 0; c < kChunks; ++c)
+#pragma unroll
+            for (int kg = 0; kg < 2; ++kg) {
+                float x8[8];
+#pragma unroll
+                for (int e = 0; e < 8; ++e) x8[e] = xq[c][8 * kg + e];
+                split8(x8, xp, bhi[c][kg], blo[c][kg]);
+            }
+        f32x16 ug[kNT];
+        first_layer<true>(ghi, glo, lds + kLdsW1, lb, gp / down1, lane, h, ug);
+        const float undo1 = down1 * ginv;
+        float dot = 0.0f, dot_v = 0.0f;
+        f32x16 prev;
+#pragma unroll
+        for (int t = 0; t < kNT; ++t) {
+            const float* unext = t + 1 < kNT ? uhrow + 32 * (t + 1) : nuhrow;
+            float b4[4][4], v4[4][4];
+            load4(lbh + 32 * t, b4[0]);
+            load4(lvh + 32 * t, v4[0]);
+            f32x16 acc;
+            second_layer_tile(bhi, blo, lds, t, lane, acc, [&](int n) {
+                if (n < 16) {
+                    const int gq = n >> 2, r = n & 3;
+                    if (r == 0 && gq + 1 < 4) {
+                        load4(lbh + 32 * t + 8 * (gq + 1), b4[gq + 1]);
+                        load4(lvh + 32 * t + 8 * (gq + 1), v4[gq + 1]);
+                    }
+                    const float x = fmaxf(fmaf(ug[t][n], undo1, un[gq][r] + b4[gq][r]), 0.0f);
+                    ug[t][n] = x;
+                    dot_v = fmaf(x, v4[gq][r], dot_v);
+                    if (r == 3) load4(unext + 8 * gq + 4 * h, un[gq]);
+                } else if (t > 0) {
+                    const int r = 2 * (n - 16);
+                    dot = fmaf(ug[t - 1][r], prev[r], dot);
+                    dot = fmaf(ug[t - 1][r + 1], prev[r + 1], dot);
+                }
+            });
+            prev = acc;
+        }
+#pragma unroll
+        for (int r = 0; r < 16; ++r) dot = fmaf(ug[kNT - 1][r], prev[r], dot);
+        dot = fmaf(dot, down2 * xinv, dot_u + dot_v);
+        dot += __shfl_xor(dot, 32, 64);
+        dot += lb[4 * kD + 3];
+        if (h == 0 && row0 + s < S) logit[row0 + s] = dot / 16.0f;
+        g0 = ng0; g1 = ng1; uhrow = nuhrow;
     }
 }
 
@@ -89,19 +249,22 @@
     __syncthreads();
     const float* lb = lds + kW;
     const float down1 = lb[(G ? 4 : 2) * kD], down2 = lb[(G ? 4 : 2) * kD + 1];
+    if constexpr (G) {
+        const int uwave = __builtin_amdgcn_readfirstlane(wave);
+        round2_g_tiles(g, uh, lds, V, R, P, S, logit, lane, ((long)blockIdx.x * kWaves + uwave) * 32, (long)gridDim.x * kWaves * 32);
+        return;
+    } else {
     float* stage = lds + kLdsStage + wave * 32 * kStageLd;
 
     for (long row0 = ((long)blockIdx.x * kWaves + wave) * 32; row0 < S; row0 += (long)gridDim.x * kWaves * 32) {
-        float4 qs[G ? 1 : kChunks][G ? 1 : 4];
-        if constexpr (!G) {
-#pragma unroll
-            for (int it = 0; it < 4; ++it) {
-                const long row = row0 + r8 + 8 * it < S ? row0 + r8 + 8 * it : S - 1;
-#pragma unroll
-                for (int c = 0; c < kChunks; ++c) {
-                    const f32x4 v = __builtin_nontemporal_load(reinterpret_cast<const f32x4*>(qry + row * kD + 32 * c + 4 * qd));
-                    qs[c][it] = make_float4(v[0], v[1], v[2], v[3]);
-                }
+        float4 qs[kChunks][4];
+#pragma unroll
+        for (int it = 0; it < 4; ++it) {
+            const long row = row0 + r8 + 8 * it < S ? row0 + r8 + 8 * it : S - 1;
+#pragma unroll
+            for (int c = 0; c < kChunks; ++c) {
+                const f32x4 v = __builtin_nontemporal_load(reinterpret_cast<const f32x4*>(qry + row * kD + 32 * c + 4 * qd));
+                qs[c][it] = make_float4(v[0], v[1], v[2], v[3]);
             }
         }
         const long srow = row0 + s < S ? row0 + s : S - 1;
@@ -121,7 +284,7 @@
             split8(gx, gp, ghi, glo);
         }
         f32x16 ug[kNT];
-        first_layer<G>(ghi, glo, lds + kLdsW1, lb, gp / down1, lane, h, ug);
+        first_layer(ghi, glo, lds + kLdsW1, lb, gp / down1, lane, h, ug);
         const float undo1 = down1 * ginv;
         float xm = 0.0f;
 #pragma unroll
@@ -129,11 +292,7 @@
 #pragma unroll
             for (int gq = 0; gq < 4; ++gq) {
                 const float4 u = *reinterpret_cast<const float4*>(uhrow + 32 * t + 8 * gq + 4 * h);
-                float uu[4] = {u.x, u.y, u.z, u.w};
-                if constexpr (G) {
-                    const float4 b = *reinterpret_cast<const float4*>(lb + 32 * t + 8 * gq + 4 * h);
-                    uu[0] += b.x; uu[1] += b.y; uu[2] += b.z; uu[3] += b.w;
-                }
+                const float uu[4] = {u.x, u.y, u.z, u.w};
 #pragma unroll
                 for (int r = 0; r < 4; ++r) {
                     const float x = fmaxf(fmaf(ug[t][4 * gq + r], undo1, uu[r]), 0.0f);
@@ -141,73 +300,27 @@
                     xm = fmaxf(xm, x);
                 }
             }
+        xm = fmaxf(xm, __shfl_xor(xm, 32, 64));
+        float xp, xinv;
+        pow2_scale(fmaxf(xm, 1e-30f), xp, xinv);
+        f32x16 acc[kNT];
+        second_layer(ug, xp, lds, lb + kD, xp / down2, lane, h, acc);
         float dot = 0.0f;
-        if constexpr (G) {
-            const float downq = lb[4 * kD + 2];
-            f32x16 xq[kNT];
-            first_layer<true>(ghi, glo, lds + kLdsWq1, lb + 2 * kD, gp / downq, lane, h, xq);
-            const float undoq = downq * ginv;
-            const float* lu = lb + 3 * kD;
-            const float* lq = lb + 2 * kD;
-            float xqm = 0.0f, dot_u = 0.0f;
-#pragma unroll
-            for (int t = 0; t < kNT; ++t)
-#pragma unroll
-                for (int gq = 0; gq < 4; ++gq) {
-                    const float4 u = *reinterpret_cast<const float4*>(lu + 32 * t + 8 * gq + 4 * h);
-                    const float4 b = *reinterpret_cast<const float4*>(lq + 32 * t + 8 * gq + 4 * h);
-                    const float uu[4] = {u.x, u.y, u.z, u.w}, bb[4] = {b.x, b.y, b.z, b.w};
-#pragma unroll
-                    for (int r = 0; r < 4; ++r) {
-                        const float x = fmaxf(fmaf(xq[t][4 * gq + r], undoq, bb[r]), 0.0f);
-                        xq[t][4 * gq + r] = x;
-                        xqm = fmaxf(xqm, x);
-                        dot_u = fmaf(uu[r], x, dot_u);
-                    }
-                }
-            xqm = fmaxf(xqm, __shfl_xor(xqm, 32, 64));
-            float xp, xinv;
-            pow2_scale(fmaxf(xqm, 1e-30f), xp, xinv);
-            f32x16 acc[kNT];
-            second_layer<true>(xq, xp, lds, lb + kD, xp / down2, lane, h, acc);
-            const float* lv = lb + kD;
-            float dot_v = 0.0f;
-#pragma unroll
-            for (int t = 0; t < kNT; ++t)
-#pragma unroll
-                for (int gq = 0; gq < 4; ++gq) {
-                    const float4 v4 = *reinterpret_cast<const float4*>(lv + 32 * t + 8 * gq + 4 * h);
-                    const float vv[4] = {v4.x, v4.y, v4.z, v4.w};
-#pragma unroll
-                    for (int r = 0; r < 4; ++r) {
-                        dot = fmaf(ug[t][4 * gq + r], acc[t][4 * gq + r], dot);
-                        dot_v = fmaf(ug[t][4 * gq + r], vv[r], dot_v);
-                    }
-                }
-            dot = fmaf(dot, down2 * xinv, dot_u + dot_v);
-            dot += __shfl_xor(dot, 32, 64);
-            dot += lb[4 * kD + 3];
-        } else {
-            xm = fmaxf(xm, __shfl_xor(xm, 32, 64));
-            float xp, xinv;
-            pow2_scale(fmaxf(xm, 1e-30f), xp, xinv);
-            f32x16 acc[kNT];
-            second_layer(ug, xp, lds, lb + kD, xp / down2, lane, h, acc);
-#pragma unroll
-            for (int t = 0; t < kNT; ++t) {
-#pragma unroll
-                for (int it = 0; it < 4; ++it) *reinterpret_cast<float4*>(stage + (r8 + 8 * it) * kStageLd + 4 * qd) = qs[t][it];
-#pragma unroll
-                for (int gq = 0; gq < 4; ++gq) {
-                    const float4 qv = *reinterpret_cast<const float4*>(stage + s * kStageLd + 8 * gq + 4 * h);
-                    dot = fmaf(acc[t][4 * gq + 0], qv.x, dot); dot = fmaf(acc[t][4 * gq + 1], qv.y, dot);
-                    dot = fmaf(acc[t][4 * gq + 2], qv.z, dot); dot = fmaf(acc[t][4 * gq + 3], qv.w, dot);
-                }
-            }
-            dot += __shfl_xor(dot, 32, 64);
-            dot *= down2 * xinv;
-        }
+#pragma unroll
+        for (int t = 0; t < kNT; ++t) {
+#pragma unroll
+            for (int it = 0; it < 4; ++it) *reinterpret_cast<float4*>(stage + (r8 + 8 * it) * kStageLd + 4 * qd) = qs[t][it];
+#pragma unroll
+            for (int gq = 0; gq < 4; ++gq) {
+                const float4 qv = *reinterpret_cast<const float4*>(stage + s * kStageLd + 8 * gq + 4 * h);
+                dot = fmaf(acc[t][4 * gq + 0], qv.x, dot); dot = fmaf(acc[t][4 * gq + 1], qv.y, dot);
+                dot = fmaf(acc[t][4 * gq + 2], qv.z, dot); dot = fmaf(acc[t][4 * gq + 3], qv.w, dot);
+            }
+        }
+        dot += __shfl_xor(dot, 32, 64);
+        dot *= down2 * xinv;
         if (h == 0 && row0 + s < S) logit[row0 + s] = dot / 16.0f;
+    }
     }
 }
 
```
